# HTDerekLiu/surface_multigrid_code

Hardware: AMD Instinct MI355X
Metric: V-cycles/sec + fine-level SpMV GB/s (% HBM peak), 1M-vert mesh fp64 (higher is better)
Workload: dtype f64; 1 GPU; C3: bunny_15K_init x3 midpoint subdivision, 1011330 verts, 5 levels, M_bary+0.01(-L), fp64; n_verts=1011330, nnz=7079298, levels=5, smoother=gs, rhs_columns_per_gpu=1, parallelism=single GPU

## Files before the change

### surface_multigrid_code_amd/csrc/smg_cycle.cpp

```cpp
#include <hip/hip_runtime.h>

#include <algorithm>
#include <chrono>
#include <cmath>
#include <cstdarg>
#include <cstdio>
#include <cstdlib>
#include <cstring>
#include <functional>
#include <memory>
#include <numeric>
#include <string>
#include <thread>
#include <vector>

#include "smg_internal.hpp"

using namespace smg;


template <typename T>
static int ensure_vectors(smg_hierarchy* h, int k)
{
    constexpr bool fp64 = std::is_same<T, double>::value;
// ... 68 lines not shown
    if ((rc = prepare_sweep_plans(h, k, h->pre, h->post))) return rc;
    return ensure_spectral_bounds(h);
}

int smg::ensure_fp32(smg_hierarchy* h, int k)
{
    const int L = h->n_levels;
    if (h->union_m > 0) return fail(SMG_ERR_INVALID, "a union handle solves in fp64 (its coarse inverses are per-member blocks: no fp32 image)");
    if (h->coarse_sparse) return fail(SMG_ERR_INVALID, "the mixed-precision cycle is not available with a sparse coarse factorisation (coarsest level of %d unknowns)", h->nc);
    if (!h->f32_valid) {
        drop_graphs(h);
        for (int lv = 0; lv < L; lv++) {
            Level& Lv = h->lv[lv];
            if (lv < L - 1 && h->bs == 3) {
                HIPCHK(Lv.bA.ensure_f32(h->stream));
                if (Lv.gs_on_transpose) HIPCHK(Lv.bAT.ensure_f32(h->stream));
            } else if (lv < L - 1) {
                HIPCHK(Lv.dA.ensure_f32(h->stream));
                if (Lv.gs_on_transpose) HIPCHK(Lv.dAT.ensure_f32(h->stream));
            }
            if (lv >= 1) {
                HIPCHK(Lv.dP.ensure_f32(h->stream));
                HIPCHK(Lv.dPT.ensure_f32(h->stream));
            }
        }
        if (h->coarse_schur) {
            HIPCHK(h->sch.arena32.ensure((size_t)h->schur.off_C));
            HIPCHK(launch_cvt_f64_f32(h->sch.arena32.p, h->sch.arena.p, (size_t)h->schur.off_C, h->stream));
            h->sch.view.arena32 = h->sch.arena32.p;
        } else {
            HIPCHK(h->d_Ainv32.ensure((size_t)h->nc_pad * h->nc_pad));
            HIPCHK(launch_cvt_f64_f32(h->d_Ainv32.p, h->d_Ainv.p, (size_t)h->nc_pad * h->nc_pad, h->stream));
        }
        h->f32_valid = true;
    }
    return ensure_vectors<float>(h, k);
}

int smg::level_kind(const smg_hierarchy* h, int lv)
{
    if (lv < 0 || lv >= h->n_levels - 1) return LV_GS;
    switch (h->smoother) {
        case SMG_SMOOTH_JACOBI: return LV_JACOBI;
        case SMG_SMOOTH_HYBRID: return h->lv[lv].n <= h->jacobi_max_rows ? LV_JACOBI : LV_GS;
        case SMG_SMOOTH_CHEBYSHEV: return LV_CHEBY;
        case SMG_SMOOTH_HYBRID_CHEBYSHEV: return h->lv[lv].n <= h->jacobi_max_rows ? LV_CHEBY : LV_GS;
    }
    return LV_GS;
}

struct ChebyCoef { double c1, c2; };
static void cheby_coefs(double lam, double frac, int degree, std::vector<ChebyCoef>& out)
{
    out.resize((size_t)std::max(degree, 0));
    const double lmax = lam, lmin = lam * frac;
    const double theta = (lmax + lmin) / 2.0, delta = (lmax - lmin) / 2.0;
    const double sigma = theta / delta;
    double rho = 1.0 / sigma;
    for (int s = 0; s < degree; s++) {
        if (s == 0) { out[s].c1 = 0.0; out[s].c2 = 1.0 / theta; }
        else {
            const double rho_new = 1.0 / (2.0 * sigma - rho);
            out[s].c1 = rho_new * rho;
            out[s].c2 = 2.0 * rho_new / delta;
            rho = rho_new;
        }
    }
}

static inline int coarse_cols(const smg_hierarchy* h, int k) { return (h->coarse_cols > 0 && h->coarse_cols < k) ? h->coarse_cols : k; }


static const SellBuf& smoothed(const Level& L) { return L.gs_on_transpose ? L.dAT : L.dA; }

template <typename T>
static hipError_t coarse_solve(smg_hierarchy* h, Level& L, int k, const Ctrl* ctrl)
{
    LevelVecs<T>& V = vecs<T>(L);
    if constexpr (std::is_same<T, double>::value) {
        if (h->union_m > 0) return launch_blockdiag_gemv_add(h->un.view, h->d_Ainv.p, h->nc, V.b.p, V.u.p, k, ctrl, h->stream);
        if (h->coarse_sparse) return launch_sparse_coarse_solve(h->c_view, V.b.p, V.u.p, k, ctrl, h->stream);
    }
    if (h->coarse_schur) return launch_schur_solve(h->sch.view, V.b.p, V.u.p, k, ctrl, h->stream);
    return launch_dense_gemv_add(by_type<T>(h->d_Ainv.p, h->d_Ainv32.p), h->nc, h->nc_pad, V.b.p, V.u.p, coarse_cols(h, k), k, ctrl, h->stream, (T*)h->d_sympart.p);
}

template <typename T>
static hipError_t op_A(smg_hierarchy* h, Level& L, bool smoother_image, SellMode m, int s0, int s1, const T* x, const T* bb, T* y, int k, const Ctrl* ctrl,
                       const FirstColour* fc = nullptr, double omega = 1.0)
{
    if (h->bs == 3) {
        const Bsr3Dev& V = (smoother_image && L.gs_on_transpose) ? L.bAT.view : L.bA.view;
        return launch_bsr3(m, V, s0, s1 < 0 ? V.n_slices : s1, x, bb, y, k, ctrl, nullptr, nullptr, h->stream, omega, fc ? fc->c1 : 0.0, fc ? fc->update<T>() : nullptr);
    }
    const SellDev& V = smoother_image ? smoothed(L).view : L.dA.view;
    return launch_sell(m, V, s0, s1 < 0 ? V.n_slices : s1, x, bb, y, k, ctrl, nullptr, nullptr, h->stream, nullptr, fc, omega);
}

static const std::vector<int>& colour_slices(const smg_hierarchy* h, const Level& Lv)
{
    if (h->bs == 3) return (Lv.gs_on_transpose ? Lv.bAT : Lv.bA).color_slice_ptr;
    return (Lv.gs_on_transpose ? Lv.dAT : Lv.dA).color_slice_ptr;
}

template <typename T>
static int enqueue_gs(smg_hierarchy* h, int lv, const SweepPlan& sp, const T* b, T* u, int k, int iters, const Ctrl* ctrl, int first = FIRST_NONE, T* t = nullptr,
                      T* res = nullptr)
{
    Level& Lv = h->lv[lv];
    ProfGuard pg(h, "MG: relaxation");
    if (const WgsBuf* W = sp.wave) {
        for (int it = 0; it < iters; it++)
            for (size_t c = 0; c + 1 < W->color_ptr.size(); c++)
                HIPCHK(launch_wgs(W->view, W->color_ptr[c], W->color_ptr[c + 1], (const double*)b, (double*)u, k, ctrl, h->stream));
        return SMG_OK;
    }
    if (const BgsBuf* Q = sp.block) {
        for (int it = 0; it < iters; it++)
            for (size_t c = 0; c + 1 < Q->color_ptr.size(); c++)
                HIPCHK(launch_bgs(Q->view, Q->color_ptr[c], Q->color_ptr[c + 1], (const double*)b, (double*)u, k, ctrl, h->stream));
        return SMG_OK;
    }
    const std::vector<int>& cs = colour_slices(h, Lv);
    const SellDev& G = smoothed(Lv).view;
    FirstColour fr;
    fr.set_update(res);
    for (int it = first == FIRST_SWEEP ? 1 : 0; it < iters; it++)
        for (size_t c = (it == 0 && first == FIRST_LAUNCH) ? 1 : 0; c + 1 < cs.size(); c++) {
            const bool last = res && it == iters - 1 && c + 2 == cs.size();
            if (it == 1 && first == FIRST_SWEEP) HIPCHK(launch_sell(last ? SELL_GS_OOP_RES : SELL_GS_OOP, G, cs[c], cs[c + 1], t, b, u, k, ctrl, nullptr, nullptr, h->stream, nullptr, last ? &fr : nullptr));
            else if (last) HIPCHK(launch_sell(SELL_GS_RES, G, cs[c], cs[c + 1], u, b, u, k, ctrl, nullptr, nullptr, h->stream, nullptr, &fr));
            else HIPCHK(op_A<T>(h, Lv, true, SELL_GS, cs[c], cs[c + 1], u, b, u, k, ctrl));
        }
    return SMG_OK;
}

template <typename T>
static int enqueue_gs_tiled(smg_hierarchy* h, const TiledDev& plan, const T* b, T* const buf[2], int* cur, int k, const Ctrl* ctrl)
{
    ProfGuard pg(h, "MG: relaxation");
    HIPCHK(launch_tiled_gs(plan, (const double*)buf[*cur], (const double*)b, (double*)buf[1 - *cur], k, ctrl, h->stream));
    *cur ^= 1;
    return SMG_OK;
}

template <typename T>
static int enqueue_jacobi(smg_hierarchy* h, int lv, const T* b, T* const buf[2], int* cur, int k, int iters, const Ctrl* ctrl)
{
    Level& Lv = h->lv[lv];
    ProfGuard pg(h, "MG: relaxation");
    for (int it = 0; it < iters; it++) {
        HIPCHK(op_A<T>(h, Lv, true, SELL_JACOBI, 0, -1, buf[*cur], b, buf[1 - *cur], k, ctrl, nullptr, h->omega));
        *cur ^= 1;
    }
    return SMG_OK;
}

template <typename T>
static int enqueue_cheby(smg_hierarchy* h, int lv, const T* b, T* const buf[2], int* cur, int k, int iters, const Ctrl* ctrl, bool first_done = false)
{
    if (iters <= 0) return SMG_OK;
    Level& Lv = h->lv[lv];
    ProfGuard pg(h, "MG: relaxation");
    std::vector<ChebyCoef> cf;
    cheby_coefs(Lv.lam, h->cheby_fraction, iters + 1, cf);
    for (int s = first_done ? 1 : 0; s <= iters; s++) {
        FirstColour fc;
        fc.set_update(vecs<T>(Lv).d.p);
        fc.c1 = cf[s].c1;
        HIPCHK(op_A<T>(h, Lv, true, SELL_CHEBY, 0, -1, buf[*cur], b, buf[1 - *cur], k, ctrl, &fc, cf[s].c2));
        *cur ^= 1;
    }
    return SMG_OK;
}

static bool fuse_first_colour() { static const int on = env_int("SMG_FUSE_FIRST", 1); return on != 0; }
static bool resid_byproduct() { static const int on = env_int("SMG_RESID_BYPRODUCT", 1); return on != 0; }
static bool prolong_skip_first() { static const int on = env_int("SMG_PROLONG_SKIP_FIRST", 1); return on != 0; }

template <typename T>
static int enqueue_vcycle_t(smg_hierarchy* h, int lv, int k, int pre, int post, const Ctrl* ctrl, int first = FIRST_NONE)
{
    const bool first_done = first != FIRST_NONE;
    const int L = h->n_levels;
    Level& Lv = h->lv[lv];
    if (lv == L - 1) {
        ProfGuard pg(h, "MG: coarse solve");
        HIPCHK(coarse_solve<T>(h, Lv, k, ctrl));
        return SMG_OK;
    }
    Level& Lc = h->lv[lv + 1];
    LevelVecs<T>&V = vecs<T>(Lv), &Vc = vecs<T>(Lc);
    const int kind = level_kind(h, lv);
    const bool jac = kind != LV_GS;
    T* const buf[2] = {V.u.p, V.t.p};
    int cur = 0;
    const bool fp64 = std::is_same<T, double>::value;
    const SweepPlan sp_pre = sweep_plan(h, lv, k, pre, fp64, first), sp_post = sweep_plan(h, lv, k, post, fp64, FIRST_NONE);
    int rc;
    const bool byprod = fp64 && resid_byproduct() && h->bs == 1 && kind == LV_GS && sp_pre.colours() && pre >= 1 && k < 8 && !Lv.gs_on_transpose &&
                        Lv.dA.n_part > 0 && Lv.dA.color_slice_ptr.size() >= 3 && (first != FIRST_SWEEP || pre >= 2);
    if (kind == LV_JACOBI) {
        if (first_done) cur = 1;
        rc = enqueue_jacobi<T>(h, lv, V.b.p, buf, &cur, k, pre - (first_done ? 1 : 0), ctrl);
    } else if (kind == LV_CHEBY) {
        if (first_done) cur = 1;
        rc = enqueue_cheby<T>(h, lv, V.b.p, buf, &cur, k, pre, ctrl, first_done);
    } else if (sp_pre.tiled) rc = enqueue_gs_tiled<T>(h, *sp_pre.tiled, V.b.p, buf, &cur, k, ctrl);
    else rc = enqueue_gs<T>(h, lv, sp_pre, V.b.p, buf[0], k, pre, ctrl, first, buf[1], byprod ? V.r.p : nullptr);
    if (rc) return rc;
    {
        ProfGuard pg(h, "MG: residual");
        if (byprod) HIPCHK(launch_sell(SELL_RESID, Lv.dA.part_view(), 0, Lv.dA.n_part, buf[cur], V.b.p, V.r.p, k, ctrl, nullptr, nullptr, h->stream));
        else HIPCHK(op_A<T>(h, Lv, false, SELL_RESID, 0, -1, buf[cur], V.b.p, V.r.p, k, ctrl));
    }
    const SellBuf& Gc = smoothed(Lc);
    const int kind_c = level_kind(h, lv + 1);
    const bool jac_c = kind_c != LV_GS;
    const bool fuse = h->bs == 1 && sweep_plan(h, lv + 1, k, pre, fp64, FIRST_NONE).colours() && fuse_first_colour() && lv + 1 < L - 1 && pre > 0 && Gc.view.vals<T>() && (jac_c ? Gc.n_all > 0 : Gc.n_first > 0);
    const int kt = k * h->bs;
    {
        ProfGuard pg(h, "MG: restrict");
        FirstColour fc;
        if (fuse) {
            fc.diag_slot = Gc.diag_slot.p; fc.n_first = jac_c ? Gc.n_all : Gc.n_first;
            fc.val = Gc.view.val; fc.valf = Gc.view.valf;
            fc.jacobi = kind_c == LV_CHEBY ? 2 : (jac_c ? 1 : 0); fc.omega = h->omega;
            if (kind_c == LV_CHEBY) {
                std::vector<ChebyCoef> cf;
                cheby_coefs(Lc.lam, h->cheby_fraction, 1, cf);
                fc.omega = cf[0].c2;
                fc.set_update(Vc.d.p);
            }
        }
        T* init = (fuse && jac_c) ? Vc.t.p : Vc.u.p;
        HIPCHK(launch_sell(SELL_AX, Lc.dPT.view, 0, Lc.dPT.view.n_slices, V.r.p, nullptr, Vc.b.p, kt, ctrl, nullptr, nullptr, h->stream, init, fuse ? &fc : nullptr));
    }
    rc = enqueue_vcycle_t<T>(h, lv + 1, k, pre, post, ctrl, fuse ? FIRST_LAUNCH : FIRST_NONE);
    if (rc) return rc;
    {
        ProfGuard pg(h, "MG: prolong");
        int dst = cur;
        const int flips = sp_post.tiled ? 1 : kind == LV_CHEBY ? (post > 0 ? post + 1 : 0) : post;
        if ((jac || sp_post.tiled) && ((cur + flips) & 1)) dst = 1 - cur;
        if (!jac && !sp_post.tiled && cur == 1) dst = 0;
        const bool skip = prolong_skip_first() && h->bs == 1 && kind == LV_GS && sp_post.colours() && post >= 1 && Lc.dP.n_part > 0;
        const SellDev Pv = skip ? Lc.dP.part_view() : Lc.dP.view;
        HIPCHK(launch_sell(SELL_ADD, Pv, 0, Pv.n_slices, Vc.u.p, buf[cur], buf[dst], kt, ctrl, nullptr, nullptr, h->stream));
        cur = dst;
    }
    if (kind == LV_CHEBY) return enqueue_cheby<T>(h, lv, V.b.p, buf, &cur, k, post, ctrl);
    if (jac) return enqueue_jacobi<T>(h, lv, V.b.p, buf, &cur, k, post, ctrl);
    if (sp_post.tiled) return enqueue_gs_tiled<T>(h, *sp_post.tiled, V.b.p, buf, &cur, k, ctrl);
    return enqueue_gs<T>(h, lv, sp_post, V.b.p, buf[0], k, post, ctrl);
}

int smg::enqueue_vcycle(smg_hierarchy* h, int k, const Ctrl* ctrl, int first)
{
    if (h->precision == 1) return enqueue_vcycle_t<float>(h, 0, k, h->pre, h->post, ctrl);
    return enqueue_vcycle_t<double>(h, 0, k, h->pre, h->post, ctrl, first);
}

int smg::apply_A(smg_hierarchy* h, int lv, SellMode mode, const double* x, const double* b, double* y, int k, const Ctrl* ctrl)
{
    HIPCHK(op_A<double>(h, h->lv[lv], false, mode, 0, -1, x, b, y, k, ctrl));
    return SMG_OK;
}


template <typename T>
static int enqueue_relax(smg_hierarchy* h, int lv, const T* b, T* u, int k, int iters, const Ctrl* ctrl, T** res)
{
    const int kind = level_kind(h, lv);
    const SweepPlan sp = sweep_plan(h, lv, k, iters, std::is_same<T, double>::value, FIRST_NONE);
    T* const buf[2] = {u, vecs<T>(h->lv[lv]).t.p};
    int cur = 0, rc;
    if (kind == LV_GS && !sp.tiled) rc = enqueue_gs<T>(h, lv, sp, b, u, k, iters, ctrl);
    else if (kind == LV_GS) rc = enqueue_gs_tiled<T>(h, *sp.tiled, b, buf, &cur, k, ctrl);
    else if (kind == LV_CHEBY) rc = enqueue_cheby<T>(h, lv, b, buf, &cur, k, iters, ctrl);
    else rc = enqueue_jacobi<T>(h, lv, b, buf, &cur, k, iters, ctrl);
    *res = buf[cur];
    return rc;
}
static int enqueue_relax_into(smg_hierarchy* h, int lv, const double* b, double* u, int k, int iters, const Ctrl* ctrl)
{
    double* res = nullptr;
    int rc = enqueue_relax<double>(h, lv, b, u, k, iters, ctrl, &res);
    if (rc) return rc;
    if (res != u) HIPCHK(hipMemcpyAsync(u, res, (size_t)h->lv[lv].n * k * sizeof(double), hipMemcpyDeviceToDevice, h->stream));
    return SMG_OK;
}

bool smg::head_fusable(smg_hierarchy* h, int k)
{
    static const int on = env_int("SMG_FUSE_HEAD", 1);
    if (!on || h->precision != 0 || h->n_levels < 2 || h->prof_on || h->bs != 1 || h->union_m > 0) return false;
    Level& L0 = h->lv[0];
    if (L0.gs_on_transpose) return false;
    if (!sweep_plan(h, 0, k, h->pre, true, FIRST_NONE).colours()) return false;
    const int kind = level_kind(h, 0);
    return kind == LV_GS ? h->pre >= 2 : h->pre >= 1;
}

int smg::enqueue_residual_ss(smg_hierarchy* h, int k, bool fuse_decide, double* sumsq_out)
{
    Level& L0 = h->lv[0];
    int nb = 0;
    if (h->head_fuse) {
        ProfGuard pg(h, "MG: relaxation");
        const int kind = level_kind(h, 0);
        const SellDev& G = L0.dA.view;
        if (kind == LV_GS) {
            const std::vector<int>& cs = L0.dA.color_slice_ptr;
            for (size_t c = 0; c + 1 < cs.size(); c++) {
                int nbc = 0;
                HIPCHK(launch_sell(SELL_GS_HEAD, G, cs[c], cs[c + 1], L0.u.p, L0.b.p, L0.t.p, k, h->d_ctrl.p, h->d_partials.p + nb, &nbc, h->stream));
                nb += nbc;
            }
        } else if (kind == LV_JACOBI) {
            HIPCHK(launch_sell(SELL_JACOBI_HEAD, G, 0, G.n_slices, L0.u.p, L0.b.p, L0.t.p, k, h->d_ctrl.p, h->d_partials.p, &nb, h->stream, nullptr, nullptr, h->omega));
        } else {
            std::vector<ChebyCoef> cf;
            cheby_coefs(L0.lam, h->cheby_fraction, h->pre + 1, cf);
            FirstColour fc;
            fc.d = L0.d.p;
            fc.c1 = cf[0].c1;
            HIPCHK(launch_sell(SELL_CHEBY_HEAD, G, 0, G.n_slices, L0.u.p, L0.b.p, L0.t.p, k, h->d_ctrl.p, h->d_partials.p, &nb, h->stream, nullptr, &fc, cf[0].c2));
        }
        if (fuse_decide) HIPCHK(launch_ss_finalize_decide(h->d_partials.p, nb, h->d_ctrl.p, h->stream));
        else HIPCHK(launch_ss_finalize(h->d_partials.p, nb, h->d_ctrl.p, h->stream, sumsq_out));
        return SMG_OK;
    }
    ProfGuard pg(h, "MG: outer residual");
    if (h->union_m > 0) {
        if (!fuse_decide) return fail(SMG_ERR_INVALID, "a union handle runs through smg_solve / smg_solve_begin + smg_raw_outer_iteration (no split-phase iteration: its members stop one by one)");
        HIPCHK(launch_sell(SELL_RESID, L0.dA.view, 0, L0.dA.view.n_slices, L0.u.p, L0.b.p, L0.r.p, k, h->d_ctrl.p, nullptr, nullptr, h->stream));
        HIPCHK(launch_union_sumsq_decide(h->un.view, L0.r.p, L0.u.p, k, h->d_ctrl.p, h->stream));
        return SMG_OK;
    }
    if (h->precision == 1 && h->bs == 3)
        HIPCHK(launch_bsr3(SELL_RESID_BOTH, L0.bA.view, 0, L0.bA.view.n_slices, L0.u.p, L0.b.p, L0.r.p, k, h->d_ctrl.p, h->d_partials.p, &nb, h->stream));
    else if (h->precision == 1)
        HIPCHK(launch_sell(SELL_RESID_BOTH, L0.dA.view, 0, L0.dA.view.n_slices, L0.u.p, L0.b.p, L0.r.p, k, h->d_ctrl.p, h->d_partials.p, &nb, h->stream));
    else if (h->bs == 3)
        HIPCHK(launch_bsr3(SELL_RESID_SS, L0.bA.view, 0, L0.bA.view.n_slices, L0.u.p, L0.b.p, nullptr, k, h->d_ctrl.p, h->d_partials.p, &nb, h->stream));
    else
        HIPCHK(launch_sell(SELL_RESID_SS, L0.dA.view, 0, L0.dA.view.n_slices, L0.u.p, L0.b.p, nullptr, k, h->d_ctrl.p, h->d_partials.p, &nb, h->stream));
    if (fuse_decide) HIPCHK(launch_ss_finalize_decide(h->d_partials.p, nb, h->d_ctrl.p, h->stream));
    else HIPCHK(launch_ss_finalize(h->d_partials.p, nb, h->d_ctrl.p, h->stream, sumsq_out));
    return SMG_OK;
}

int smg::enqueue_cycle_part(smg_hierarchy* h, int k, const double* d_sumsq)
{
    if (d_sumsq) HIPCHK(launch_decide(h->d_ctrl.p, d_sumsq, h->stream));
    {
        ProfGuard pg(h, "MG: total VCycle");
        if (h->precision == 1) {
            Level& L0 = h->lv[0];
            const size_t cnt = (size_t)L0.n * k;
            HIPCHK(launch_residual_to_f32(L0.f32.b.p, L0.f32.u.p, L0.r.p, cnt, h->d_ctrl.p, h->stream));
            int rc = enqueue_vcycle(h, k, h->d_ctrl.p, FIRST_NONE);
            if (rc) return rc;
            HIPCHK(launch_add_correction(L0.u.p, L0.f32.u.p, cnt, h->d_ctrl.p, h->stream));
        } else {
            int rc = enqueue_vcycle(h, k, h->d_ctrl.p, h->head_fuse ? FIRST_SWEEP : FIRST_NONE);
            if (rc) return rc;
            if (h->union_m > 0) HIPCHK(launch_union_restore(h->un.view, h->lv[0].u.p, k, h->d_ctrl.p, h->stream));
        }
    }
    return SMG_OK;
}

int smg::coarse_stall_check(smg_hierarchy* h)
{
    if (!h->coarse_sparse || !h->c_err.p) return SMG_OK;
    int cerr = 0;
    HIPCHK(hipMemcpy(&cerr, h->c_err.p, sizeof(int), hipMemcpyDeviceToHost));
    if (!cerr) return SMG_OK;
    (void)hipMemset(h->c_err.p, 0, sizeof(int));
    return fail(SMG_ERR_HIP, "the triangular solves of the sparse coarse factorisation stalled (results are NaN)");
}

int smg::check_ready(const smg_hierarchy* h, const char* who)
{
    if (!h) return fail(SMG_ERR_INVALID, "%s: null handle", who);
    if (!h->precomputed) return fail(SMG_ERR_INVALID, "%s: call smg_precompute first", who);
    if (h->device < 0) return fail(SMG_ERR_NO_DEVICE, "%s: no HIP device", who);
    return SMG_OK;
}

int smg::internal_cols(const smg_hierarchy* h, int k)
{
    static const int on = env_int("SMG_PAD_COLS", 1);
    if (!on || k <= 4 || k > 64 || h->union_m > 0) return k;
    if (k > 32) return k > 40 ? 64 : k;
    int p = 8;
    while (p < k) p *= 2;
    return p;
}

static int piece_prolog(smg_hierarchy* h, int lv, int k, const char* who, bool need_coarser);

static int time_graph(smg_hierarchy* h, hipGraphExec_t g, int reps, double* us)
{
    hipEvent_t e0, e1;
    HIPCHK(hipEventCreate(&e0));
    HIPCHK(hipEventCreate(&e1));
    for (int i = 0; i < 3; i++) HIPCHK(hipGraphLaunch(g, h->stream));
    HIPCHK(hipEventRecord(e0, h->stream));
    for (int i = 0; i < reps; i++) HIPCHK(hipGraphLaunch(g, h->stream));
    HIPCHK(hipEventRecord(e1, h->stream));
    HIPCHK(hipStreamSynchronize(h->stream));
    float ms = 0.f;
    HIPCHK(hipEventElapsedTime(&ms, e0, e1));
    *us = 1e3 * ms / reps;
    (void)hipEventDestroy(e0); (void)hipEventDestroy(e1); (void)hipGraphExecDestroy(g);
    return SMG_OK;
}

extern "C" int smg_bench_vcycle(smg_hierarchy* h, int lv, int k, int pre, int post, int reps, double* us_per_cycle)
{
    int rc = piece_prolog(h, lv, k, "smg_bench_vcycle", false);
    if (rc) return rc;
    DeviceScope dsc(h->device);
    if (reps < 1 || !us_per_cycle) return fail(SMG_ERR_INVALID, "smg_bench_vcycle: bad arguments");
    if ((rc = prepare_sweep_plans(h, k, pre, post))) return rc;
    hipGraphExec_t g = nullptr;
    rc = capture_graph(h, &g, [&]() { return enqueue_vcycle_t<double>(h, lv, k, pre, post, nullptr); });
    if (rc) return rc;
    if ((rc = time_graph(h, g, reps, us_per_cycle))) return rc;
    return coarse_stall_check(h);
}

extern "C" int smg_bench_relax(smg_hierarchy* h, int lv, int k, int sweeps, int reps, double* us_per_call)
{
    int rc = piece_prolog(h, lv, k, "smg_bench_relax", true);
    if (rc) return rc;
    DeviceScope dsc(h->device);
    if (reps < 1 || sweeps < 1 || !us_per_call) return fail(SMG_ERR_INVALID, "smg_bench_relax: bad arguments");
    if ((rc = prepare_sweep_plans(h, k, sweeps, sweeps))) return rc;
    Level& Lv = h->lv[lv];
    hipGraphExec_t g = nullptr;
    rc = capture_graph(h, &g, [&]() { return enqueue_relax_into(h, lv, Lv.b.p, Lv.u.p, k, sweeps, nullptr); });
    if (rc) return rc;
    return time_graph(h, g, reps, us_per_call);
}

extern "C" int smg_synchronize(smg_hierarchy* h)
// ... 414 lines not shown
```

### surface_multigrid_code_amd/csrc/smg_device.hip

```cpp
#include <hip/hip_runtime.h>

#include <cstdlib>
#include <type_traits>

#include "smg_device.hpp"
#include "smg_device_inl.hpp"
#include "smg_gj_inl.hpp"

namespace smg {


__device__ int g_never_done = 0;
const int* never_done()
{
    static const int* p = nullptr;
    if (!p) { void* q = nullptr; if (hipGetSymbolAddress(&q, HIP_SYMBOL(g_never_done)) == hipSuccess) p = (const int*)q; }
    return p;
}


template <typename T> struct CoarseInit { T* u; const T* gs_val; const int* diag_slot; int n_first; int jacobi; T omega; T* d; T c1; int codes; T tab[4]; };
template <typename T> __device__ __forceinline__ T code_val(const CoarseInit<T>& z, int cw)
{
    const T lo = (cw & 1) ? z.tab[1] : z.tab[0], hi = (cw & 1) ? z.tab[3] : z.tab[2];
    return (cw & 2) ? hi : lo;
}

template <int MODE, int KB, typename T, int W0C = -1, int WPB = 4, bool CODED = false>
__global__ __launch_bounds__(64 * WPB) void k_sell(const int* a_col, const T* a_val, const int* a_order, const int* a_slice_off, int a_stride,
                                              int a_w_lo, int s_begin, int s_end, int n_blocks, int use_order, const T* x,
                                              const int* a_slice_row, const int* a_slice_w, const T* b, T* y, int ld, const int* done,
                                              double* partials, CoarseInit<T> z)
{
    struct { const int *slice_row, *slice_off, *slice_w, *order, *col; int stride, w_lo; } A = {a_slice_row, a_slice_off, a_slice_w, a_order,
                                                                                               a_col, a_stride, a_w_lo};
    constexpr int C = 64;
    const int lane = threadIdx.x & 63;
    const int wave = threadIdx.x >> 6;
    constexpr int wpb = WPB;
    constexpr bool GS = sell_is_gs(MODE), OOP = sell_is_oop(MODE), JAC = sell_is_jacobi(MODE), CHEB = sell_is_cheby(MODE), HEAD = sell_is_head(MODE);
    constexpr bool RES = sell_has_res(MODE);
    int bid;
    if (GS && n_blocks < 0) { if (blockIdx.x & 7) return; bid = blockIdx.x >> 3; }
    else bid = xcd_remap(blockIdx.x, n_blocks);
    const int ls = __builtin_amdgcn_readfirstlane(s_begin + bid * wpb + wave);
    double ss = 0.0;
    int stop = 0;
    if (ls < s_end) {
        const int s = (!GS && use_order) ? A.order[ls] : ls;
        const int W0 = W0C >= 0 ? W0C : (A.w_lo < 8 ? A.w_lo : 8);
        const int off0 = (W0C >= 0 || A.stride) ? s * A.stride : A.slice_off[s];
        const int* cp = A.col + (size_t)off0 * C + lane;
        const T* vp = CODED ? nullptr : a_val + (size_t)off0 * C + lane;
        constexpr int U = W0C > 8 ? W0C : 8;
        int c0[U];
        T v0[U];
#pragma unroll
        for (int t = 0; t < U; t++) {
            if (t < W0) { c0[t] = cp[(size_t)t * C]; v0[t] = CODED ? (T)0 : vp[(size_t)t * C]; }
            else { c0[t] = -1; v0[t] = (T)0; }
        }
        {
            size_t keep = (size_t)x ^ (size_t)A.slice_row ^ (size_t)A.slice_w ^ (size_t)b ^ (size_t)y ^ (size_t)done ^ (size_t)ld;
            if (MODE == SELL_AX) keep ^= (size_t)z.u ^ (size_t)z.gs_val ^ (size_t)z.diag_slot ^ (size_t)z.n_first ^ (size_t)z.jacobi ^ (size_t)z.d;
            if (CHEB || RES) keep ^= (size_t)z.d;
            asm("" : "+s"(keep));
            if (keep == 0x5a5a5a5a5a5a5a5bull) return;
        }
        stop = load_flag(done);
        const int row0 = A.slice_row[s];
        const int nrow = A.slice_row[s + 1] - row0;
        const int w = A.slice_w[s];
        const int rowb = row0 + lane;
        const int split = OOP ? A.slice_row[s_begin] : 0;
        T acc[KB];
        T accr[KB];
        T diag = (T)1;
        T xi[KB];
        T dold[KB];
        T bv[KB];
        const bool live = lane < nrow;
        T zd = (T)1;
        if (MODE == SELL_AX && live && rowb < z.n_first) zd = z.gs_val[z.diag_slot[rowb]];
#pragma unroll
        for (int q = 0; q < KB; q++) {
            acc[q] = (T)0; accr[q] = (T)0; xi[q] = (T)0; dold[q] = (T)0;
            if (MODE == SELL_AX) bv[q] = (T)0;
            else bv[q] = live ? b[(size_t)rowb * ld + q] : (T)0;
            if (CHEB && live && z.c1 != (T)0) dold[q] = z.d[(size_t)rowb * ld + q];
        }
        bool has_diag = false;
        auto consume = [&](const int (&cw)[U], const T (&vw)[U]) {
            int c[U];
            T v[U];
#pragma unroll
            for (int t = 0; t < U; t++) {
                if constexpr (CODED) { c[t] = cw[t] >> 2; v[t] = code_val<T>(z, cw[t]); }
                else { c[t] = cw[t]; v[t] = vw[t]; }
            }
            T xv[U][KB];
            T xo[MODE == SELL_GS_HEAD ? U : 1][KB];
#pragma unroll
            for (int t = 0; t < U; t++) {
                const bool use = (c[t] >= 0) && !(GS && c[t] == rowb);
                if constexpr (MODE == SELL_GS_HEAD) {
                    gather_kb<KB, T>(x + (size_t)c[t] * ld, c[t] >= 0, xo[t]);
                    gather_kb<KB, T>((const T*)y + (size_t)c[t] * ld, use && c[t] < split, xv[t]);
                } else if constexpr (MODE == SELL_GS_OOP || MODE == SELL_GS_OOP_RES) {
                    gather_kb<KB, T>((c[t] < split ? (const T*)y : x) + (size_t)c[t] * ld, use, xv[t]);
                } else {
                    gather_kb<KB, T>(x + (size_t)c[t] * ld, use, xv[t]);
                }
            }
#pragma unroll
            for (int t = 0; t < U; t++) {
                if (c[t] >= 0) {
                    if (HEAD) {
#pragma unroll
                        for (int q = 0; q < KB; q++) accr[q] += v[t] * (MODE == SELL_GS_HEAD ? xo[t][q] : xv[t][q]);
                    }
                    if (GS && c[t] == rowb) {
                        diag = v[t];
                        if (RES) has_diag = true;
                    } else if ((JAC || CHEB) && c[t] == rowb) {
// ... 413 lines not shown
        else if (A.w_max <= 16) SMG_WIDE_LAT(16);
        else SMG_WIDE_LAT(32);
#undef SMG_WIDE_LAT
        *nb_out = nb;
        return;
    }
    const int waves = ns * (KW / 2);
    const int nb = (waves + 3) / 4;
    hipLaunchKernelGGL((k_sell_wide<MODE, KW, T>), dim3(nb), dim3(256), 0, st, A.col, A.vals<T>(), A.order, A.slice_off, A.stride, s_begin, s_end, nb, use_order, x,
                       A.slice_row, A.slice_w, b, y, k, done, partials, zero_rows);
    *nb_out = nb;
}

int sell_wide_blocks(int n_slices, int k)
{
    int tot = 0, c0 = 0;
    while (k - c0 >= 8) { int kw = 64; while (kw > k - c0) kw >>= 1; tot += (n_slices * kw + 3) / 4; c0 += kw; }
    return tot;
}

static constexpr int sell_wpb() { return 4; }
static int gs_wpb() { static const int v = getenv("SMG_GS_WPB") ? atoi(getenv("SMG_GS_WPB")) : 4; return v; }
int sell_blocks(int n_slices) { return (n_slices + sell_wpb() - 1) / sell_wpb(); }

template <typename T>
struct NarrowRun {
    int s_begin, s_end, use_order;
    const T *xx, *bb;
    T* yy;
    int k;
    const int* done;
    double* pp;
    const CoarseInit<T>& zz;
    hipStream_t st;
};
template <int MODE, int KB, typename T, int W0C, int WPB, bool CODED>
static void narrow_one(const SellDev& A, int grid, int nbarg, const NarrowRun<T>& R)
{
    hipLaunchKernelGGL((k_sell<MODE, KB, T, W0C, WPB, CODED>), dim3(grid), dim3(64 * WPB), 0, R.st, A.col, CODED ? nullptr : A.vals<T>(), A.order, A.slice_off, A.stride, A.w_lo,
                       R.s_begin, R.s_end, nbarg, R.use_order, R.xx, A.slice_row, A.slice_w, R.bb, R.yy, R.k, R.done, R.pp, R.zz);
}
template <int MODE, typename T, bool CODED>
static void launch_narrow(const SellDev& A, int kb, int nb, int ns, int grid, int nbarg, bool one_xcd, const NarrowRun<T>& R)
{
    static_assert(sell_wpb() == 4, "the narrow kernels below are instantiated for 4 waves per workgroup");
    const bool w7 = A.stride > 0 && A.w_lo == 7;
    switch (kb) {
        case 1: {
            const int w0 = A.stride > 0 ? (A.w_lo < 8 ? A.w_lo : 8) : -1;
            static const int pitch_env = getenv("SMG_PITCH_SPEC_MAX") ? atoi(getenv("SMG_PITCH_SPEC_MAX")) : -1;
            const int pitch_max = pitch_env >= 0 ? pitch_env : (sell_is_gs(MODE) ? 32 : 64);
            if (nb <= pitch_max && A.stride == 12 && w0 >= 7) narrow_one<MODE, 1, T, 12, 4, CODED>(A, grid, nbarg, R);
            else if (!CODED && w0 == 7 && MODE == SELL_GS && !one_xcd && gs_wpb() == 8) narrow_one<SELL_GS, 1, T, 7, 8, false>(A, (ns + 7) / 8, (ns + 7) / 8, R);
            else if (!CODED && w0 == 7 && MODE == SELL_GS && !one_xcd && gs_wpb() == 2) narrow_one<SELL_GS, 1, T, 7, 2, false>(A, (ns + 1) / 2, (ns + 1) / 2, R);
            else if (w0 == 7) narrow_one<MODE, 1, T, 7, 4, CODED>(A, grid, nbarg, R);
            else if (w0 == 8) narrow_one<MODE, 1, T, 8, 4, CODED>(A, grid, nbarg, R);
            else if (w0 == 2) narrow_one<MODE, 1, T, 2, 4, CODED>(A, grid, nbarg, R);
            else narrow_one<MODE, 1, T, -1, 4, CODED>(A, grid, nbarg, R);
            break;
        }
        case 2:
            if (w7) narrow_one<MODE, 2, T, 7, 4, CODED>(A, grid, nbarg, R);
            else narrow_one<MODE, 2, T, -1, 4, CODED>(A, grid, nbarg, R);
            break;
        case 3:
            if (w7) narrow_one<MODE, 3, T, 7, 4, CODED>(A, grid, nbarg, R);
            else narrow_one<MODE, 3, T, -1, 4, CODED>(A, grid, nbarg, R);
            break;
        default:
            if (w7) narrow_one<MODE, 4, T, 7, 4, CODED>(A, grid, nbarg, R);
            else narrow_one<MODE, 4, T, -1, 4, CODED>(A, grid, nbarg, R);
            break;
    }
}

template <int MODE, typename T>
static hipError_t launch_sell_mode(const SellDev& A, int s_begin, int s_end_in, const T* x, const T* b, T* y,
                                   int k, const Ctrl* ctrl, double* partials, int* n_blocks, hipStream_t st, T* zero_rows, const FirstColour* first,
                                   double omega)
{
    int s_end = s_end_in;
    if (MODE == SELL_ADD && !b) b = y;
    if constexpr (sell_has_res(MODE)) { if (k >= 8 || !first || !first->d || zero_rows || s_end_in != A.n_slices) return hipErrorInvalidValue; }
    const int ns = s_end - s_begin;
    const int nb = sell_blocks(ns);
    const int* done = ctrl ? &ctrl->done : never_done();
    static const int dbg_empty = getenv("SMG_DEBUG_EMPTY") ? atoi(getenv("SMG_DEBUG_EMPTY")) : 0;
    if (dbg_empty == 1) s_end = s_begin;
    const int use_order = (A.order && s_begin == 0 && s_end == A.n_slices) ? 1 : 0;
    if (n_blocks) *n_blocks = 0;
    if (ns <= 0) return hipSuccess;
    int c0 = 0;
    size_t poff = 0;
    if constexpr (!sell_has_res(MODE)) {
        while (k - c0 >= 8) {
            int kw = 64;
            while (kw > k - c0) kw >>= 1;
            const T* xx = x ? x + c0 : nullptr;
            const T* bb = b ? b + c0 : nullptr;
            T* yy = y ? y + c0 : nullptr;
            double* pp = partials ? partials + poff : nullptr;
            const CoarseInit<T> zz = coarse_codes<T>(A, zero_rows, c0, first, omega);
            int wnb = 0;
            switch (kw) {
                case 64: launch_wide_one<MODE, 64, T>(A, s_begin, s_end, use_order, xx, bb, yy, k, done, pp, zz, st, &wnb); break;
                case 32: launch_wide_one<MODE, 32, T>(A, s_begin, s_end, use_order, xx, bb, yy, k, done, pp, zz, st, &wnb); break;
                case 16: launch_wide_one<MODE, 16, T>(A, s_begin, s_end, use_order, xx, bb, yy, k, done, pp, zz, st, &wnb); break;
                default: launch_wide_one<MODE, 8, T>(A, s_begin, s_end, use_order, xx, bb, yy, k, done, pp, zz, st, &wnb); break;
            }
            poff += (size_t)wnb;
            c0 += kw;
        }
    }
    static const int one_xcd_max = getenv("SMG_ONE_XCD_MAX") ? atoi(getenv("SMG_ONE_XCD_MAX")) : 32;
    const bool one_xcd = sell_is_gs(MODE) && nb <= one_xcd_max;
    const int grid = one_xcd ? nb * 8 : nb, nbarg = one_xcd ? -nb : nb;
    for (; c0 < k; c0 += 4) {
        const int kb = (k - c0) < 4 ? (k - c0) : 4;
        const T* xx = x ? x + c0 : nullptr;
        const T* bb = b ? b + c0 : nullptr;
        T* yy = y ? y + c0 : nullptr;
        double* pp = partials ? partials + poff : nullptr;
        const CoarseInit<T> zz = coarse_codes<T>(A, zero_rows, c0, first, omega);
        poff += (size_t)nb;
        if constexpr (std::is_same<T, double>::value && (MODE == SELL_AX || MODE == SELL_RESID)) {
            int kd = kb;
            if (kd == 4 && !deep_wanted(MODE, A.w_max, 4) && deep_wanted(MODE, A.w_max, 2)) kd = 2;
            if (deep_wanted(MODE, A.w_max, kd) || (kd > 1 && deep_wanted(MODE, A.w_max, 1))) {
                for (int cc = 0; cc < kb;) {
                    int kk = kb - cc;
                    while (kk > 1 && !deep_wanted(MODE, A.w_max, kk)) kk--;
                    const int nbm = A.w_max <= 24 ? 3 : A.w_max <= 40 ? 5 : 8;
                    const CoarseInit<T> zc = coarse_codes<T>(A, zero_rows, c0 + cc, first, omega);
#define SMG_DEEP_LAUNCH(KB, NB) hipLaunchKernelGGL((k_sell_deep<MODE, KB, NB>), dim3(nb), dim3(256), 0, st, A.col, A.val, A.order, A.slice_off, A.stride, s_begin, s_end, nb, use_order, \
                                                   xx ? xx + cc : nullptr, A.slice_row, A.slice_w, bb ? bb + cc : nullptr, yy + cc, k, done, zc)
                    if (nbm == 3) { if (kk == 1) SMG_DEEP_LAUNCH(1, 3); else if (kk == 2) SMG_DEEP_LAUNCH(2, 3); else SMG_DEEP_LAUNCH(3, 3); }
                    else if (nbm == 5) { if (kk == 1) SMG_DEEP_LAUNCH(1, 5); else SMG_DEEP_LAUNCH(2, 5); }
                    else SMG_DEEP_LAUNCH(1, 8);
#undef SMG_DEEP_LAUNCH
                    cc += kk;
                }
                continue;
            }
        }
        const NarrowRun<T> run{s_begin, s_end, use_order, xx, bb, yy, k, done, pp, zz, st};
        if constexpr (MODE == SELL_AX || MODE == SELL_ADD) {
            if (A.codes) { launch_narrow<MODE, T, true>(A, kb, nb, ns, grid, nbarg, one_xcd, run); continue; }
        }
        launch_narrow<MODE, T, false>(A, kb, nb, ns, grid, nbarg, one_xcd, run);
    }
    if (MODE == SELL_AX && A.long_n > 0 && s_begin == 0 && s_end_in == A.n_slices && A.long_vals<T>()) {
        const CoarseInit<T> zz = coarse_codes<T>(A, zero_rows, 0, first, omega);
        if (k >= 8) {
            const long waves = (long)A.long_n * ((k + 63) / 64);
            hipLaunchKernelGGL((k_long_ax_cols<T>), dim3((unsigned)((waves + 3) / 4)), dim3(256), 0, st, A.long_row, A.long_ptr, A.long_col, A.long_vals<T>(), A.long_n, x, y,
                               k, k, done, zz);
        } else {
            const long waves = (long)A.long_n * k;
            hipLaunchKernelGGL((k_long_ax<T>), dim3((unsigned)((waves + 3) / 4)), dim3(256), 0, st, A.long_row, A.long_ptr, A.long_col, A.long_vals<T>(), A.long_n, x, y, k, k,
                               done, zz);
        }
    }
    if (n_blocks) *n_blocks = (int)poff;
    return hipGetLastError();
}

template <typename T>
static hipError_t launch_sell_any(SellMode mode, const SellDev& A, int s_begin, int s_end, const T* x, const T* b,
                                  T* y, int k, const Ctrl* ctrl, double* partials, int* n_blocks, hipStream_t st,
                                  T* zero_rows, const FirstColour* first, double omega)
{
    constexpr bool fp64 = std::is_same<T, double>::value;
    if (!fp64 && ((!A.valf && !A.codes) || partials)) return hipErrorInvalidValue;
    switch (mode) {
#define SMG_SELL_CASE(M) \
        case M: \
            if constexpr (fp64 || !sell_fp64_only(M)) return launch_sell_mode<M, T>(A, s_begin, s_end, x, b, y, k, ctrl, partials, n_blocks, st, zero_rows, first, omega); \
            else return hipErrorInvalidValue;
        SMG_SELL_CASE(SELL_JACOBI) SMG_SELL_CASE(SELL_CHEBY) SMG_SELL_CASE(SELL_AX) SMG_SELL_CASE(SELL_RESID) SMG_SELL_CASE(SELL_RESID_SS)
        SMG_SELL_CASE(SELL_ADD) SMG_SELL_CASE(SELL_GS) SMG_SELL_CASE(SELL_RESID_BOTH) SMG_SELL_CASE(SELL_GS_OOP) SMG_SELL_CASE(SELL_GS_HEAD)
        SMG_SELL_CASE(SELL_JACOBI_HEAD) SMG_SELL_CASE(SELL_CHEBY_HEAD) SMG_SELL_CASE(SELL_GS_RES) SMG_SELL_CASE(SELL_GS_OOP_RES)
#undef SMG_SELL_CASE
    }
    return hipErrorInvalidValue;
}

hipError_t launch_sell(SellMode mode, const SellDev& A, int s_begin, int s_end, const double* x, const double* b,
                       double* y, int k, const Ctrl* ctrl, double* partials, int* n_blocks, hipStream_t st,
                       double* zero_rows, const FirstColour* first, double omega)
{
    return launch_sell_any<double>(mode, A, s_begin, s_end, x, b, y, k, ctrl, partials, n_blocks, st, zero_rows, first, omega);
}
hipError_t launch_sell(SellMode mode, const SellDev& A, int s_begin, int s_end, const float* x, const float* b,
                       float* y, int k, const Ctrl* ctrl, double* partials, int* n_blocks, hipStream_t st,
                       float* zero_rows, const FirstColour* first, double omega)
{
    return launch_sell_any<float>(mode, A, s_begin, s_end, x, b, y, k, ctrl, partials, n_blocks, st, zero_rows, first, omega);
}

__global__ __launch_bounds__(256) void k_gershgorin(const int* a_col, const double* a_val, const int* a_slice_row, const int* a_slice_off, const int* a_slice_w,
                                                    int stride, int n_slices, unsigned long long* out)
{
    const int lane = threadIdx.x & 63, s = blockIdx.x * 4 + (threadIdx.x >> 6);
    double ratio = 0.0;
    if (s < n_slices) {
        const int row0 = a_slice_row[s], nrow = a_slice_row[s + 1] - row0, w = a_slice_w[s];
        const size_t off = (size_t)(stride ? s * stride : a_slice_off[s]) * 64 + lane;
        double sum = 0.0, diag = 0.0;
        for (int j = 0; j < w; j++) {
            const int c = a_col[off + (size_t)j * 64];
            const double v = a_val[off + (size_t)j * 64];
            if (c >= 0) { sum += fabs(v); if (c == row0 + lane) diag = v; }
        }
        if (lane < nrow && diag > 0.0) ratio = sum / diag;
    }
#pragma unroll
    for (int o = 32; o > 0; o >>= 1) ratio = fmax(ratio, __shfl_down(ratio, o, 64));
    if (lane == 0 && ratio > 0.0) atomicMax(out, (unsigned long long)__double_as_longlong(ratio));
}
hipError_t launch_gershgorin(const SellDev& A, double* out, hipStream_t st)
{
    hipError_t e = hipMemsetAsync(out, 0, sizeof(double), st);
    if (e != hipSuccess || A.n_slices <= 0) return e;
    hipLaunchKernelGGL(k_gershgorin, dim3((A.n_slices + 3) / 4), dim3(256), 0, st, A.col, A.val, A.slice_row, A.slice_off, A.slice_w, A.stride, A.n_slices,
                       (unsigned long long*)out);
    return hipGetLastError();
}


__global__ __launch_bounds__(256) void k_ss_finalize(const double* partials, int n, Ctrl* ctrl, double* out)
{
    if (ctrl->done) return;
    __shared__ double red[256];
    double s = 0.0;
    for (int i = threadIdx.x; i < n; i += 256) s += partials[i];
    red[threadIdx.x] = s;
    __syncthreads();
    for (int o = 128; o > 0; o >>= 1) {
        if ((int)threadIdx.x < o) red[threadIdx.x] += red[threadIdx.x + o];
        __syncthreads();
    }
    if (threadIdx.x == 0) *out = red[0];
}

__global__ __launch_bounds__(256) void k_ss_finalize_decide(const double* partials, int n, Ctrl* ctrl)
{
    __shared__ double red[256];
    const int done = ctrl->done, n_his = ctrl->n_his, his_cap = ctrl->his_cap;
    const double tol = ctrl->tol;
    double* const r_his = ctrl->r_his;
    double s = 0.0;
#pragma unroll 8
    for (int i = threadIdx.x; i < n; i += 256) s += partials[i];
    if (done) return;
    red[threadIdx.x] = s;
    __syncthreads();
    for (int o = 128; o > 0; o >>= 1) {
        if ((int)threadIdx.x < o) red[threadIdx.x] += red[threadIdx.x + o];
        __syncthreads();
    }
    if (threadIdx.x == 0) {
        const double sumsq = red[0], r = sqrt(sumsq);
        ctrl->sumsq = sumsq;
        if (n_his < his_cap) r_his[n_his] = r;
        ctrl->n_his = n_his + 1;
        ctrl->r_prev = ctrl->r_last; ctrl->r_last = r;
        if (!(r == r) || r > 1.7e308) { ctrl->status = -1; ctrl->done = 1; }
        else if (r < tol) ctrl->done = 1;
    }
}

__global__ void k_decide(Ctrl* ctrl, const double* sumsq)
{
    if (ctrl->done) return;
    decide_body(ctrl, *sumsq);
}

constexpr int SS_STAGE_MIN = 16384, SS_STAGE_WGS = 128;
__global__ __launch_bounds__(256) void k_ss_stage(const double* __restrict__ partials, int n, double* __restrict__ out, const int* done)
{
    if (load_flag(done)) return;
    __shared__ double red[256];
    const int per = (n + SS_STAGE_WGS - 1) / SS_STAGE_WGS;
    const int i0 = blockIdx.x * per, i1 = min(n, i0 + per);
    double s = 0.0;
#pragma unroll 8
    for (int i = i0 + (int)threadIdx.x; i < i1; i += 256) s += partials[i];
    red[threadIdx.x] = s;
    __syncthreads();
    for (int o = 128; o > 0; o >>= 1) {
        if ((int)threadIdx.x < o) red[threadIdx.x] += red[threadIdx.x + o];
        __syncthreads();
    }
    if (threadIdx.x == 0) out[blockIdx.x] = red[0];
}
static const double* ss_stage(const double* partials, int& n, const Ctrl* ctrl, hipStream_t st)
{
    if (n < SS_STAGE_MIN) return partials;
    double* out = const_cast<double*>(partials) + n;
    hipLaunchKernelGGL(k_ss_stage, dim3(SS_STAGE_WGS), dim3(256), 0, st, partials, n, out, &ctrl->done);
    n = SS_STAGE_WGS;
    return out;
}
int ss_partials_room() { return SS_STAGE_WGS; }

hipError_t launch_ss_finalize(const double* partials, int n, Ctrl* ctrl, hipStream_t st, double* out)
{
    partials = ss_stage(partials, n, ctrl, st);
    hipLaunchKernelGGL(k_ss_finalize, dim3(1), dim3(256), 0, st, partials, n, ctrl, out ? out : &ctrl->sumsq);
    return hipGetLastError();
}
__global__ void k_decide_spec(Ctrl* ctrl, const double* sumsq)
{
    ctrl->just_done = 0;
    if (ctrl->done) return;
    decide_body(ctrl, *sumsq);
    if (ctrl->done) ctrl->just_done = 1;
}
__global__ void k_copy_unless_done(double* dst, const double* src, size_t n, const int* done)
{
    if (*done) return;
    const size_t i = (size_t)blockIdx.x * blockDim.x + threadIdx.x;
    if (i < n) dst[i] = src[i];
}
__global__ void k_restore_if_just_done(double* dst, const double* src, size_t n, const Ctrl* ctrl)
{
    if (!ctrl->just_done) return;
    const size_t i = (size_t)blockIdx.x * blockDim.x + threadIdx.x;
    if (i < n) dst[i] = src[i];
}
hipError_t launch_decide_spec(Ctrl* ctrl, const double* sumsq, hipStream_t st)
{
    hipLaunchKernelGGL(k_decide_spec, dim3(1), dim3(1), 0, st, ctrl, sumsq);
    return hipGetLastError();
}
hipError_t launch_copy_unless_done(double* dst, const double* src, size_t n, const Ctrl* ctrl, hipStream_t st)
{
    if (n == 0) return hipSuccess;
    hipLaunchKernelGGL(k_copy_unless_done, dim3((unsigned)((n + 255) / 256)), dim3(256), 0, st, dst, src, n, &ctrl->done);
    return hipGetLastError();
}
hipError_t launch_restore_if_just_done(double* dst, const double* src, size_t n, const Ctrl* ctrl, hipStream_t st)
{
    if (n == 0) return hipSuccess;
    hipLaunchKernelGGL(k_restore_if_just_done, dim3((unsigned)((n + 255) / 256)), dim3(256), 0, st, dst, src, n, ctrl);
    return hipGetLastError();
}
hipError_t launch_ss_finalize_decide(const double* partials, int n, Ctrl* ctrl, hipStream_t st)
{
    partials = ss_stage(partials, n, ctrl, st);
    hipLaunchKernelGGL(k_ss_finalize_decide, dim3(1), dim3(256), 0, st, partials, n, ctrl);
    return hipGetLastError();
}
hipError_t launch_decide(Ctrl* ctrl, const double* sumsq, hipStream_t st)
{
    hipLaunchKernelGGL(k_decide, dim3(1), dim3(1), 0, st, ctrl, sumsq);
    return hipGetLastError();
}

template <typename T> struct Vec2;
template <> struct Vec2<double> { typedef double type __attribute__((ext_vector_type(2))); };
template <> struct Vec2<float> { typedef float type __attribute__((ext_vector_type(2))); };

template <int KB, typename T>
__global__ __launch_bounds__(256) void k_dense_gemv_add(const T* __restrict__ Ainv, int n, int lda,
                                                        const T* __restrict__ b, T* u, int ld, const int* done)
{
    const int stop = load_flag(done);
    const int lane = threadIdx.x & 63;
    const int row = blockIdx.x * 4 + (threadIdx.x >> 6);
    if (row >= n) return;
    using T2 = typename Vec2<T>::type;
    const T2* a2 = reinterpret_cast<const T2*>(Ainv + (size_t)row * lda);
    T acc[KB];
#pragma unroll
    for (int q = 0; q < KB; q++) acc[q] = (T)0;
    const int n2 = lda >> 1;
#pragma unroll 4
    for (int jj = lane; jj < n2; jj += 64) {
        const T2 a = a2[jj];
#pragma unroll
        for (int q = 0; q < KB; q++) {
            acc[q] += a.x * b[(size_t)(2 * jj) * ld + q];
            acc[q] += a.y * b[(size_t)(2 * jj + 1) * ld + q];
        }
    }
#pragma unroll
// ... 142 lines not shown
            for (int c = 0; c < CPW; c++) bn[c][t] = (q < per && col0 + 16 * c + lc < kvalid) ? pb[q * sb + 16 * c] : 0.0;
        }
#pragma unroll
        for (int t = 0; t < DEPTH; t++)
#pragma unroll
            for (int c = 0; c < CPW; c++) acc[c] = __builtin_amdgcn_mfma_f64_16x16x4f64(av[t], bv[c][t], acc[c], 0, 0, 0);
#pragma unroll
        for (int t = 0; t < DEPTH; t++) {
            av[t] = an[t];
#pragma unroll
            for (int c = 0; c < CPW; c++) bv[c][t] = bn[c][t];
        }
    }
    __shared__ double red[CPW][4][4][64];
#pragma unroll
    for (int c = 0; c < CPW; c++)
#pragma unroll
        for (int r = 0; r < 4; r++) red[c][w][r][lane] = acc[c][r];
    __syncthreads();
    if (!stop) {
        for (int c = w; c < CPW; c += 4) {
#pragma unroll
            for (int r = 0; r < 4; r++) {
                const int row = row0 + lr + 4 * r;
                if (row < n && col0 + 16 * c + lc < kvalid) {
                    const size_t o = (size_t)row * ld + col0 + 16 * c + lc;
                    u[o] = u[o] + ((red[c][0][r][lane] + red[c][1][r][lane]) + (red[c][2][r][lane] + red[c][3][r][lane]));
                }
            }
        }
    }
}

template <typename T>
__global__ __launch_bounds__(256) void k_sym_gemv_tiles(const T* __restrict__ Ainv, int lda, const T* __restrict__ b, T* __restrict__ part, int nb)
{
    const int idx = blockIdx.x;
    int I = (int)((sqrtf(8.0f * (float)idx + 1.0f) - 1.0f) * 0.5f);
    I -= (I * (I + 1) / 2 > idx);
    I += ((I + 1) * (I + 2) / 2 <= idx);
    const int J = idx - I * (I + 1) / 2;
    __shared__ T tile[64][65];
    __shared__ T bI[64], bJ[64];
    const int t = threadIdx.x;
#pragma unroll
    for (int e = 0; e < 16; e++) {
        const int idx = e * 256 + t, r = idx >> 6, c = idx & 63;
        tile[r][c] = Ainv[(size_t)(I * 64 + r) * lda + J * 64 + c];
    }
    if (t < 64) bJ[t] = b[J * 64 + t];
    else if (t < 128) bI[t - 64] = b[I * 64 + t - 64];
    __syncthreads();
    __shared__ T red[4][64];
    const int g = t >> 6, l = t & 63, h0 = (g & 1) * 32;
    T s = (T)0;
    if (g < 2) {
#pragma unroll 8
        for (int c = h0; c < h0 + 32; c++) s += tile[l][c] * bJ[c];
    } else {
#pragma unroll 8
        for (int r = h0; r < h0 + 32; r++) s += tile[r][l] * bI[r];
    }
    red[g][l] = s;
    __syncthreads();
    if (t < 64) part[((size_t)I * nb + J) * 64 + t] = red[0][t] + red[1][t];
    else if (t < 128 && I != J) part[((size_t)J * nb + I) * 64 + (t - 64)] = red[2][t - 64] + red[3][t - 64];
}
template <typename T>
__global__ __launch_bounds__(256) void k_sym_gemv_sum(const T* __restrict__ part, int nb, int n, T* u, const int* done)
{
    const int stop = load_flag(done);
    __shared__ T red[4][64];
    const int a = blockIdx.x, g = threadIdx.x >> 6, l = threadIdx.x & 63;
    const int q = (nb + 3) / 4, b0 = g * q, b1 = min(nb, b0 + q);
    T s = (T)0;
#pragma unroll 8
    for (int bidx = b0; bidx < b1; bidx++) s += part[((size_t)a * nb + bidx) * 64 + l];
    red[g][l] = s;
    __syncthreads();
    const int i = a * 64 + l;
    if (g == 0 && i < n && !stop) u[i] = u[i] + ((red[0][l] + red[1][l]) + (red[2][l] + red[3][l]));
}

template <typename T>
static hipError_t launch_dense_T(const T* Ainv, int n, int lda, const T* b, T* u, int k, int ld, const Ctrl* ctrl, hipStream_t st, void* sym_work)
{
    const int* done = ctrl ? &ctrl->done : never_done();
    const int nb = (n + 3) / 4;
    if (n <= 0) return hipSuccess;
    if (k == 1 && ld == 1 && sym_work && lda % 64 == 0 && lda >= 512) {
        const int nt = lda / 64;
        hipLaunchKernelGGL((k_sym_gemv_tiles<T>), dim3(nt * (nt + 1) / 2), dim3(256), 0, st, Ainv, lda, b, (T*)sym_work, nt);
        hipLaunchKernelGGL((k_sym_gemv_sum<T>), dim3(nt), dim3(256), 0, st, (const T*)sym_work, nt, n, u, done);
        return hipGetLastError();
    }
    int c0 = 0;
    static const int use_mfma8 = getenv("SMG_COARSE_MFMA") ? atoi(getenv("SMG_COARSE_MFMA")) : 1;
    const int mfma_min = (std::is_same<T, double>::value && use_mfma8 && lda % 64 == 0) ? 8 : 16;
    while (k - c0 >= mfma_min) {
        int kc = 64;
        while (kc > k - c0 && kc > 16) kc >>= 1;
        const int kv = kc < k - c0 ? kc : k - c0;
        const int tb = (n + 15) / 16;
        static const int use_mfma = getenv("SMG_COARSE_MFMA") ? atoi(getenv("SMG_COARSE_MFMA")) : 1;
        if constexpr (std::is_same<T, double>::value) {
            if (use_mfma && lda % 64 == 0) {
                static const int cpw = getenv("SMG_COARSE_CPW") ? atoi(getenv("SMG_COARSE_CPW")) : 2;
                if (kc == 64 && cpw == 2) { hipLaunchKernelGGL((k_dense_gemm_mfma_multi<64, 2>), dim3(tb * 2), dim3(256), 0, st, Ainv, n, lda, b + c0, u + c0, ld, done, kv); c0 += kv; continue; }
                switch (kc) {
                    case 64: hipLaunchKernelGGL((k_dense_gemm_mfma<64>), dim3(tb * 4), dim3(256), 0, st, Ainv, n, lda, b + c0, u + c0, ld, done, kv); break;
                    case 32: hipLaunchKernelGGL((k_dense_gemm_mfma<32>), dim3(tb * 2), dim3(256), 0, st, Ainv, n, lda, b + c0, u + c0, ld, done, kv); break;
                    default: hipLaunchKernelGGL((k_dense_gemm_mfma<16>), dim3(tb), dim3(256), 0, st, Ainv, n, lda, b + c0, u + c0, ld, done, kv); break;
                }
                c0 += kv;
                continue;
            }
        }
        switch (kc) {
            case 64: hipLaunchKernelGGL((k_dense_gemm_tile<64, T>), dim3(tb), dim3(256), 0, st, Ainv, n, lda, b + c0, u + c0, ld, done); break;
            case 32: hipLaunchKernelGGL((k_dense_gemm_tile<32, T>), dim3(tb), dim3(256), 0, st, Ainv, n, lda, b + c0, u + c0, ld, done); break;
            default: hipLaunchKernelGGL((k_dense_gemm_tile<16, T>), dim3(tb), dim3(256), 0, st, Ainv, n, lda, b + c0, u + c0, ld, done); break;
        }
        c0 += kc;
    }
    for (; c0 < k; c0 += 4) {
        const int kb = (k - c0) < 4 ? (k - c0) : 4;
        switch (kb) {
            case 1: hipLaunchKernelGGL((k_dense_gemv_add<1, T>), dim3(nb), dim3(256), 0, st, Ainv, n, lda, b + c0, u + c0, ld, done); break;
            case 2: hipLaunchKernelGGL((k_dense_gemv_add<2, T>), dim3(nb), dim3(256), 0, st, Ainv, n, lda, b + c0, u + c0, ld, done); break;
            case 3: hipLaunchKernelGGL((k_dense_gemv_add<3, T>), dim3(nb), dim3(256), 0, st, Ainv, n, lda, b + c0, u + c0, ld, done); break;
            default: hipLaunchKernelGGL((k_dense_gemv_add<4, T>), dim3(nb), dim3(256), 0, st, Ainv, n, lda, b + c0, u + c0, ld, done); break;
        }
    }
    return hipGetLastError();
}
template <typename T>
static hipError_t launch_sym_tiles_T(const T* Ainv, int lda, const T* b, T* part, hipStream_t st)
{
    if (lda <= 0 || lda % 64) return hipErrorInvalidValue;
    const int nt = lda / 64;
    hipLaunchKernelGGL((k_sym_gemv_tiles<T>), dim3(nt * (nt + 1) / 2), dim3(256), 0, st, Ainv, lda, b, part, nt);
    return hipGetLastError();
}
hipError_t launch_sym_gemv_tiles(const double* Ainv, int lda, const double* b, double* part, hipStream_t st) { return launch_sym_tiles_T<double>(Ainv, lda, b, part, st); }
hipError_t launch_sym_gemv_tiles(const float* Ainv, int lda, const float* b, float* part, hipStream_t st) { return launch_sym_tiles_T<float>(Ainv, lda, b, part, st); }
hipError_t launch_dense_gemv_add(const double* Ainv, int n, int lda, const double* b, double* u, int k, int ld,
                                 const Ctrl* ctrl, hipStream_t st, double* sym_work)
{
    return launch_dense_T<double>(Ainv, n, lda, b, u, k, ld, ctrl, st, sym_work);
}
hipError_t launch_dense_gemv_add(const float* Ainv, int n, int lda, const float* b, float* u, int k, int ld,
                                 const Ctrl* ctrl, hipStream_t st, float* sym_work)
{
    return launch_dense_T<float>(Ainv, n, lda, b, u, k, ld, ctrl, st, sym_work);
}

__global__ void k_cvt_f64_f32(float* dst, const double* src, size_t n)
{
    const size_t i = (size_t)blockIdx.x * blockDim.x + threadIdx.x;
    if (i < n) dst[i] = (float)src[i];
}
__global__ void k_residual_to_f32(float* b32, float* u32, const double* r64, size_t n, const int* done)
{
    if (done && *done) return;
    const size_t i = (size_t)blockIdx.x * blockDim.x + threadIdx.x;
    if (i < n) { b32[i] = (float)r64[i]; u32[i] = 0.0f; }
}
__global__ void k_add_correction(double* z, const float* e, size_t n, const int* done)
{
    if (done && *done) return;
    const size_t i = (size_t)blockIdx.x * blockDim.x + threadIdx.x;
    if (i < n) z[i] = z[i] + (double)e[i];
}
hipError_t launch_cvt_f64_f32(float* dst, const double* src, size_t n, hipStream_t st)
{
    if (n == 0) return hipSuccess;
    hipLaunchKernelGGL(k_cvt_f64_f32, dim3((unsigned)((n + 255) / 256)), dim3(256), 0, st, dst, src, n);
    return hipGetLastError();
}
hipError_t launch_residual_to_f32(float* b32, float* u32, const double* r64, size_t n, const Ctrl* ctrl, hipStream_t st)
{
    if (n == 0) return hipSuccess;
    hipLaunchKernelGGL(k_residual_to_f32, dim3((unsigned)((n + 255) / 256)), dim3(256), 0, st, b32, u32, r64, n, ctrl ? &ctrl->done : nullptr);
    return hipGetLastError();
}
hipError_t launch_add_correction(double* z, const float* e, size_t n, const Ctrl* ctrl, hipStream_t st)
{
    if (n == 0) return hipSuccess;
    hipLaunchKernelGGL(k_add_correction, dim3((unsigned)((n + 255) / 256)), dim3(256), 0, st, z, e, n, ctrl ? &ctrl->done : nullptr);
    return hipGetLastError();
}

constexpr int GJ_H = 32;

__global__ __launch_bounds__(256) void k_gj_diag(const double* M, int n, int kb, double* dinv)
{
    __shared__ double a[GJ_NB][GJ_NB + 1];
    __shared__ double Rb[16][GJ_NB + 1];
    __shared__ double Cb[GJ_NB][17];
    const int K = kb * GJ_NB;
    for (int e = threadIdx.x; e < GJ_NB * GJ_NB; e += 256) a[e / GJ_NB][e % GJ_NB] = M[(size_t)(K + e / GJ_NB) * n + K + e % GJ_NB];
    __syncthreads();
    gj_invert64(a, Rb, Cb);
    for (int e = threadIdx.x; e < GJ_NB * GJ_NB; e += 256) dinv[e] = a[e / GJ_NB][e % GJ_NB];
}

__global__ __launch_bounds__(256) void k_gj_panels(const double* M, int n, int kb, const double* dinv, double* rowp,
                                                   double* colp)
{
    __shared__ double m_s[GJ_NB][GJ_H + 1];
    const int K = kb * GJ_NB;
    const int j0 = blockIdx.x * GJ_H;
    const int J = j0 / GJ_NB;
    const int t = threadIdx.x;
    if (J == kb) {
        for (int e = t; e < GJ_NB * GJ_H; e += 256) {
            const int r = e / GJ_H, c = e % GJ_H;
            rowp[(size_t)r * n + j0 + c] = dinv[r * GJ_NB + j0 + c - K];
        }
        return;
    }
    const int lane = t & 63, w = t >> 6, lr = lane >> 4, lc = lane & 15;
    double av[GJ_NB / 4], mr[8];
#pragma unroll
    for (int q = 0; q < GJ_NB / 4; q++) av[q] = dinv[(16 * w + lc) * GJ_NB + 4 * q + lr];
    if (J < kb) {
#pragma unroll
        for (int e = 0; e < 8; e++) { const int x = t + 256 * e; mr[e] = M[(size_t)(K + x / GJ_H) * n + j0 + x % GJ_H]; }
#pragma unroll
        for (int e = 0; e < 8; e++) { const int x = t + 256 * e; m_s[x / GJ_H][x % GJ_H] = mr[e]; }
    } else {
#pragma unroll
        for (int e = 0; e < 8; e++) { const int x = t + 256 * e; mr[e] = M[(size_t)(j0 + x / GJ_NB) * n + K + x % GJ_NB]; }
#pragma unroll
        for (int e = 0; e < 8; e++) { const int x = t + 256 * e; m_s[x % GJ_NB][x / GJ_NB] = mr[e]; }
    }
    __syncthreads();
// ... 607 lines not shown
```

### surface_multigrid_code_amd/csrc/smg_device.hpp

```cpp
#pragma once
#include <hip/hip_runtime_api.h>

#include <cstdint>
#include <type_traits>

namespace smg {

template <typename T, typename D, typename F>
constexpr auto by_type(D d, F f) { if constexpr (std::is_same<T, double>::value) return d; else return f; }

struct Ctrl {
    int done;
    int n_his;
    int status;
    int just_done;
    double sumsq;
    double tol;
    double* r_his;
    int his_cap;
    int pad_;
    double r_last, r_prev;
};

struct SellDev {
    int n_rows = 0, n_cols = 0, n_slices = 0;
    int C = 64;
    const int* slice_row = nullptr;
    const int* slice_off = nullptr;
    const int* slice_w = nullptr;
    int stride = 0;
    int w_lo = 0;
    int w_max = 0;
    const int* order = nullptr;
    const int* col = nullptr;
    const double* val = nullptr;
    const float* valf = nullptr;
    int codes = 0;
    double tab[4] = {0.0, 0.0, 0.0, 0.0};
    float tabf[4] = {0.0f, 0.0f, 0.0f, 0.0f};
    int long_n = 0;
    const int* long_row = nullptr;
    const int* long_ptr = nullptr;
    const int* long_col = nullptr;
    const double* long_val = nullptr;
    const float* long_valf = nullptr;
    template <typename T> const T* vals() const { return by_type<T>(val, valf); }
    template <typename T> const T* long_vals() const { return by_type<T>(long_val, long_valf); }
    template <typename T> const T* table() const { return by_type<T>(tab, tabf); }
};

enum SellMode {
    SELL_AX = 0,
    SELL_RESID = 1,
    SELL_RESID_SS = 2,
    SELL_ADD = 3,
    SELL_GS = 4,
    SELL_RESID_BOTH = 5,
    SELL_JACOBI = 6,
    SELL_CHEBY = 7,
    SELL_GS_OOP = 8,
    SELL_GS_HEAD = 9,
    SELL_JACOBI_HEAD = 10,
    SELL_CHEBY_HEAD = 11,
    SELL_GS_RES = 12,
    SELL_GS_OOP_RES = 13,
};
constexpr bool sell_has_res(int m) { return m == SELL_GS_RES || m == SELL_GS_OOP_RES; }
constexpr bool sell_is_gs(int m) { return m == SELL_GS || m == SELL_GS_OOP || m == SELL_GS_HEAD || sell_has_res(m); }
constexpr bool sell_is_oop(int m) { return m == SELL_GS_OOP || m == SELL_GS_HEAD || m == SELL_GS_OOP_RES; }
constexpr bool sell_is_jacobi(int m) { return m == SELL_JACOBI || m == SELL_JACOBI_HEAD; }
constexpr bool sell_is_cheby(int m) { return m == SELL_CHEBY || m == SELL_CHEBY_HEAD; }
constexpr bool sell_is_head(int m) { return m == SELL_GS_HEAD || m == SELL_JACOBI_HEAD || m == SELL_CHEBY_HEAD; }
constexpr bool sell_has_ss(int m) { return sell_is_head(m) || m == SELL_RESID_SS || m == SELL_RESID_BOTH; }
constexpr bool sell_fp64_only(int m) { return sell_has_ss(m) || sell_is_oop(m) || sell_has_res(m); }

struct FirstColour {
    const int* diag_slot = nullptr;
    int n_first = 0;
    const double* val = nullptr;
    const float* valf = nullptr;
    int jacobi = 0;
    double omega = 1.0;
    double* d = nullptr;
    float* df = nullptr;
    double c1 = 0.0;
    template <typename T> const T* vals() const { return by_type<T>(val, valf); }
    template <typename T> T* update() const { return by_type<T>(d, df); }
    template <typename T> void set_update(T* p) { if constexpr (std::is_same<T, double>::value) d = p; else df = p; }
};
hipError_t launch_sell(SellMode mode, const SellDev& A, int s_begin, int s_end, const double* x, const double* b,
                       double* y, int k, const Ctrl* ctrl, double* partials, int* n_blocks, hipStream_t st,
                       double* zero_rows = nullptr, const FirstColour* first = nullptr, double omega = 1.0);
hipError_t launch_sell(SellMode mode, const SellDev& A, int s_begin, int s_end, const float* x, const float* b,
                       float* y, int k, const Ctrl* ctrl, double* partials, int* n_blocks, hipStream_t st,
                       float* zero_rows = nullptr, const FirstColour* first = nullptr, double omega = 1.0);
hipError_t launch_gershgorin(const SellDev& A, double* out, hipStream_t st);
struct Bsr3Dev {
    int n_vert = 0, n_slices = 0, w_max = 0;
    const int* slice_row = nullptr;
    const int* slice_off = nullptr;
    const int* slice_w = nullptr;
    const int* order = nullptr;
    const int* col = nullptr;
    const double* val = nullptr;
    const float* valf = nullptr;
    template <typename T> const T* vals() const { return by_type<T>(val, valf); }
};
hipError_t launch_bsr3(SellMode mode, const Bsr3Dev& A, int s_begin, int s_end, const double* x, const double* b, double* y, int k, const Ctrl* ctrl,
                       double* partials, int* n_blocks, hipStream_t st, double omega = 1.0, double c1 = 0.0, double* dvec = nullptr);
hipError_t launch_bsr3(SellMode mode, const Bsr3Dev& A, int s_begin, int s_end, const float* x, const float* b, float* y, int k, const Ctrl* ctrl,
                       double* partials, int* n_blocks, hipStream_t st, double omega = 1.0, double c1 = 0.0, float* dvec = nullptr);
hipError_t launch_bsr3_gershgorin(const Bsr3Dev& A, double* out, hipStream_t st);
int bsr3_blocks(int n_slices);
hipError_t launch_bsr3_fill(const int* ptr, const int* col, const double* val, const int* gptr, const int* gcol, const int* perm, const int* iperm, const Bsr3Dev& B,
                            size_t panel_cols, bool transposed, hipStream_t st);

struct BgsDev {
    int n_blocks = 0, n_colors = 0, xrows = 0;
    const int* hdr = nullptr;
    const int* xrow = nullptr;
    const int* ugrow = nullptr;
    const int* ulrow = nullptr;
    const double* udiag = nullptr;
    const int* eidx = nullptr;
    const double* eval = nullptr;
};
hipError_t launch_bgs(const BgsDev& P, int b_begin, int b_end, const double* b, double* u, int k, const Ctrl* ctrl, hipStream_t st);

struct WgsDev {
    int n_pieces = 0, n_colors = 0, rim_pitch = 0, nb_max = 0;
    const int* hdr = nullptr;
    const int* grow = nullptr;
    const int* meta = nullptr;
    const double* diag = nullptr;
    const int* rim = nullptr;
    const unsigned* eoff = nullptr;
    const double* eval = nullptr;
};
hipError_t launch_wgs(const WgsDev& P, int q_begin, int q_end, const double* b, double* u, int k, const Ctrl* ctrl, hipStream_t st);

struct UnionDev {
    int m = 0, his_cap = 0, max_rows = 0;
    const int* rows = nullptr;
    const int* rptr = nullptr;
    const int* crow_member = nullptr;
    const long long* moff = nullptr;
    const int* mlda = nullptr;
    const int* mrow0 = nullptr;
    double* ss = nullptr;
    double* his = nullptr;
    int* nhis = nullptr;
    int* done = nullptr;
    double* zsave = nullptr;
};
hipError_t launch_blockdiag_gemv_add(const UnionDev& U, const double* Ainv, int n, const double* b, double* u, int k, const Ctrl* ctrl, hipStream_t st);
hipError_t launch_union_sumsq_decide(const UnionDev& U, const double* r, const double* u, int k, Ctrl* ctrl, hipStream_t st);
hipError_t launch_union_restore(const UnionDev& U, double* u, int k, const Ctrl* ctrl, hipStream_t st);
hipError_t launch_scatter_dense(double* dense, const double* src, const long long* pos, int nnz, hipStream_t st);
hipError_t launch_dense_identity(double* dense, int np, int n, hipStream_t st);

struct TiledDev {
    int n_tiles = 0, nc = 0, P = 0, sweeps = 0, max_ext = 0, w_max = 0, threads = 512;
    const int* hdr = nullptr;
    const int* ext_rows = nullptr;
    const int* pcol = nullptr;
    const double* pval = nullptr;
    const int* prow = nullptr;
    const double* pdiag = nullptr;
};
hipError_t launch_tiled_gs(const TiledDev& T, const double* x, const double* b, double* y, int k, const Ctrl* ctrl, hipStream_t st);
hipError_t tiled_gs_prepare(int max_ext);

struct SparseCholDev {
    int n = 0;
    const int* perm = nullptr;
    const int *rptr = nullptr, *rcol = nullptr;
    const int *cptr = nullptr, *crow = nullptr;
    const double *rval = nullptr, *cval = nullptr, *diag = nullptr;
    double* work = nullptr;
    int* err = nullptr;
};
hipError_t launch_sparse_coarse_solve(const SparseCholDev& F, const double* b, double* u, int k, const Ctrl* ctrl, hipStream_t st);
int sparse_coarse_work_cols(int k);

constexpr int SCHUR_M_MAX_DEV = 128;
struct SchurDev {
    int n = 0, nb = 0, ns = 0, ns_pad = 0;
    const int *irow = nullptr, *bsize = nullptr, *srow = nullptr, *sptr = nullptr, *sidx = nullptr, *aptr = nullptr, *ablk = nullptr, *apan = nullptr;
    double* arena = nullptr;
    float* arena32 = nullptr;
    long long off_D = 0, off_P = 0, off_W = 0, off_S = 0, off_C = 0;
    const long long *coff = nullptr, *pos = nullptr, *pos2 = nullptr, *ones = nullptr, *rdst = nullptr, *rdst2 = nullptr, *rsrc = nullptr;
    const int* rptr = nullptr;
    int nnz = 0, n_ones = 0, n_red = 0;
    double *g = nullptr, *xs = nullptr;
    float *g32 = nullptr, *xs32 = nullptr;
    double* sym_work = nullptr;
    double* gj_work = nullptr;
    template <typename T> const T* factors() const { return by_type<T>(arena, arena32); }
    template <typename T> T* rhs() const { return by_type<T>(g, g32); }
    template <typename T> T* sol() const { return by_type<T>(xs, xs32); }
};
hipError_t launch_schur_factor(const SchurDev& F, const double* vals, hipStream_t st);
hipError_t launch_schur_check(const SchurDev& F, int* d_flag, hipStream_t st);
hipError_t launch_schur_solve(const SchurDev& F, const double* b, double* u, int k, const Ctrl* ctrl, hipStream_t st);
hipError_t launch_schur_solve(const SchurDev& F, const float* b, float* u, int k, const Ctrl* ctrl, hipStream_t st);

int sell_blocks(int n_slices);
int sell_wide_blocks(int n_slices, int k);

int ss_partials_room();
hipError_t launch_ss_finalize(const double* partials, int n, Ctrl* ctrl, hipStream_t st, double* out = nullptr);
hipError_t launch_decide(Ctrl* ctrl, const double* sumsq, hipStream_t st);
hipError_t launch_decide_spec(Ctrl* ctrl, const double* sumsq, hipStream_t st);
hipError_t launch_copy_unless_done(double* dst, const double* src, size_t n, const Ctrl* ctrl, hipStream_t st);
hipError_t launch_restore_if_just_done(double* dst, const double* src, size_t n, const Ctrl* ctrl, hipStream_t st);
hipError_t launch_ss_finalize_decide(const double* partials, int n, Ctrl* ctrl, hipStream_t st);

enum { KS_RZ = 0, KS_RZ_PREV = 1, KS_ALPHA = 2, KS_BETA = 3, KS_SLOTS = 4 };
constexpr int KRY_MAX_GROUPS = 512;
struct KryDev {
    int n = 0, k = 0;
    int groups = 0;
    double* part = nullptr;
    double* s = nullptr;
    int* restart = nullptr;
};
int kry_groups(int n, int k);
hipError_t launch_kry_dots_zr_zq(const KryDev& K, const double* z, const double* r, const double* q, const Ctrl* ctrl, hipStream_t st);
hipError_t launch_kry_direction(const KryDev& K, const double* z, double* p, const Ctrl* ctrl, hipStream_t st);
hipError_t launch_kry_dots_pq(const KryDev& K, const double* p, const double* q, const Ctrl* ctrl, hipStream_t st);
hipError_t launch_kry_step_decide(const KryDev& K, double* x, double* r, const double* p, const double* q, Ctrl* ctrl, hipStream_t st);
hipError_t launch_kry_precond_in(const double* r, double* b0, double* u0, size_t cnt, const Ctrl* ctrl, hipStream_t st);
hipError_t launch_kry_widen(const float* e, double* z, size_t cnt, const Ctrl* ctrl, hipStream_t st);
hipError_t launch_kry_arm(const KryDev& K, Ctrl* ctrl, bool reopen, hipStream_t st);

struct EigBlocks {
    const double* p[3] = {nullptr, nullptr, nullptr};
    int nb = 0;
};
constexpr int EIG_TILE = 64;
constexpr int EIG_MAX_GROUPS = 256;
int eig_groups(int n);
size_t eig_gram_part_size(int a, int b, int groups);
hipError_t launch_eig_gram(const EigBlocks& Sa, const EigBlocks& Sb, int n, int m, const double* w, bool sym, double* part, int groups,
                           double* G, const Ctrl* ctrl, hipStream_t st);
hipError_t launch_eig_combine(const EigBlocks& S, const EigBlocks& AS, int n, int m, const double* C, double* X, double* AX, double* P,
                              double* AP, const Ctrl* ctrl, hipStream_t st);
hipError_t launch_eig_residual(const double* X, const double* AX, const double* mass, const double* lam, int n, int m, double* b0, double* u0,
                               float* b32, float* u32, double* part, int groups, double* res, const Ctrl* ctrl, hipStream_t st);

hipError_t launch_dense_gemv_add(const double* Ainv, int n, int lda, const double* b, double* u, int k, int ld,
                                 const Ctrl* ctrl, hipStream_t st, double* sym_work = nullptr);
hipError_t launch_dense_gemv_add(const float* Ainv, int n, int lda, const float* b, float* u, int k, int ld,
                                 const Ctrl* ctrl, hipStream_t st, float* sym_work = nullptr);
hipError_t launch_sym_gemv_tiles(const double* Ainv, int lda, const double* b, double* part, hipStream_t st);
hipError_t launch_sym_gemv_tiles(const float* Ainv, int lda, const float* b, float* part, hipStream_t st);
hipError_t launch_cvt_f64_f32(float* dst, const double* src, size_t n, hipStream_t st);
hipError_t launch_residual_to_f32(float* b32, float* u32, const double* r64, size_t n, const Ctrl* ctrl, hipStream_t st);
hipError_t launch_add_correction(double* z, const float* e, size_t n, const Ctrl* ctrl, hipStream_t st);
hipError_t launch_spd_inverse(double* M, int n, double* work, hipStream_t st);

hipError_t launch_recipe(int n_out, const int* ptr, const int* idx, const double* coef, const double* src, double* out, hipStream_t st);
hipError_t launch_sell_fill(const int* ptr, const int* col, const double* val, const int* perm, const int* iperm, const SellDev& S, size_t padded, hipStream_t st,
                            bool transposed = false);
hipError_t launch_sell_encode(const SellDev& S, size_t padded, const double* tab, int n_tab, int* out_col, int* bad, hipStream_t st);
hipError_t launch_sell_diag_slots(const SellDev& S, int* slot, int* first_missing, hipStream_t st);
hipError_t warm_device_code(hipStream_t st);
hipError_t launch_sell_fill_map(const int* ptr, const int* col, const int* perm, const int* iperm, const SellDev& S, size_t padded, bool transposed, int* map, hipStream_t st);
hipError_t launch_bit_symmetric(int n, const int* ptr, const int* col, const double* val, int* differs, hipStream_t st);
hipError_t launch_gather_vals(double* dst, const double* src, const int* map, size_t n, hipStream_t st);
hipError_t launch_dense_from_csr(double* dense, int np, int n, const double* src, const long long* pos, int nnz, hipStream_t st);
hipError_t launch_add_at(double* v, const int* where, int n, double c, hipStream_t st);

hipError_t launch_assemble(int nV, int nF, int nnz, const double* V, const int* F, int voronoi, const int* l_ptr, const int* l_idx,
                           const signed char* l_sgn, const int* m_ptr, const int* m_idx, const int* diag_of, double* Qc, double* Qm,
                           double* Md, double mass_coef, double lap_coef, double* val, double* Lval, hipStream_t st);

hipError_t launch_gather_in(double* dst, const double* src, const int* map, int n, int k, int kin, int ld_src,
                            hipStream_t st);
hipError_t launch_scatter_out(double* dst, const double* src, const int* map, int n, int k, int kin, int ld_dst,
                              hipStream_t st);
hipError_t launch_scatter_cm(double* dst, const double* src, const int* idx, int n, int k, int ld_src, int ld_dst,
                             hipStream_t st);
hipError_t launch_gather_cm(double* dst, const double* src, const int* idx, int n, int k, int ld_src, int ld_dst,
                            hipStream_t st);
hipError_t launch_csr_sub(int n_rows, const int* ptr, const int* col, const double* val, const double* x, int ldx,
                          double* y, int ld, int k, hipStream_t st);

hipError_t launch_geo_basis(const double* V, const int* F, int nF, double* W, double* Af, hipStream_t st);
hipError_t launch_geo_scatter(int n, int k, const int* src_ptr, const int* src, double* B, int ldb, hipStream_t st);
hipError_t launch_geo_divergence(int n, int k, const int* F, const double* W, const double* Af, const int* m_ptr, const int* m_idx,
                                 const double* U, int ldu, double* out, int ldo, hipStream_t st);
hipError_t launch_geo_shift(int n, int k, const int* src_ptr, const int* src, const double* phi, int ldp, double* mean, double* D, int ldd,
                            hipStream_t st);

hipError_t launch_arap_covariance(int n, const int* rowptr, const int* col, const double* w, const double* P0, const double* P, double* S, hipStream_t st);
hipError_t launch_arap_rotations(int n, const int* rowptr, const int* col, const double* w, const double* P0, const double* P, double* R, double* eterm,
                                 hipStream_t st);
hipError_t launch_arap_vertex_energy(int n, const int* rowptr, const int* col, const double* w, const double* P0, const double* P, const double* R,
                                     double* eterm, hipStream_t st);
hipError_t launch_arap_rhs(int n, const int* rowptr, const int* col, const double* w, const double* P0, const double* R, double* B, int ldb, hipStream_t st);
hipError_t launch_arap_rows(int n, const double* U, int ldu, double* P, hipStream_t st);
hipError_t launch_arap_columns(int n, const double* P, double* U, int ldu, hipStream_t st);
hipError_t launch_arap_set_handles(int nh, const int* handles, const double* hp, int ldh, double* U, int ldu, hipStream_t st);

int fixed_sum_groups(int n);
hipError_t launch_fixed_sum(const double* term, int n, double* part, double* sum, hipStream_t st);

hipError_t launch_membrane_rest(int nF, const int* F, const double* V0, double thickness, double* rest, hipStream_t st);
hipError_t launch_membrane_faces(int mode, int nF, const int* F, const double* P, const double* rest, double alpha, double beta, double floor,
                                 double value, double* W, double* G, double* H, hipStream_t st);
hipError_t launch_membrane_matrix(int nB, const int* brow, const int* bcol, const int* bptr, const int* c_ptr, const int* c_src, const double* H,
                                  int nF, double dt2, const double* mass0, double mass_scale, double* val, hipStream_t st);
hipError_t launch_membrane_pressure(int nV, int nF, const int* F, const double* P, const int* m_ptr, const int* m_idx, double pressure, double* Qn,
                                    double* mass, double* fext, hipStream_t st);
hipError_t launch_membrane_gradient(int nV, const int* m_ptr, const int* m_idx, const double* G, int nF, const double* mass0, double mass_scale,
                                    double dt, const double* qdot, const double* qdot0, const double* fext, double* g, double* b, hipStream_t st);
hipError_t launch_membrane_trial(int nV, const double* qdot, const double* dx, double step, const double* qdot0, const double* pos0,
                                 const double* fext, const double* mass0, double mass_scale, double dt, double* t_out, double* p_out, double* term,
                                 hipStream_t st);
hipError_t launch_membrane_dot3(int nV, const double* a, const double* b, double* term, hipStream_t st);

}
```

### surface_multigrid_code_amd/csrc/smg_hier.hpp

```cpp
#pragma once
#include <memory>
#include <hip/hip_runtime_api.h>

#include <atomic>
#include <cstdint>
#include <string>
#include <vector>

#include "smg_bsr3.hpp"
#include "smg_coarse.hpp"
#include "smg_device.hpp"
#include "smg_mesh.hpp"
#include "smg_order.hpp"
#include "smg_sparse.hpp"
#include "smg_tiled.hpp"
#include "smg_bgs.hpp"
#include "smg_wgs.hpp"
#include "smg_schur.hpp"

namespace smg {

inline std::atomic<long long>& devbuf_live_bytes() { static std::atomic<long long> v{0}; return v; }

template <typename T>
// ... 163 lines not shown
    BgsBuf bgs;
    std::vector<int> A_int_src;
    DevBuf<double> d_Aval;
    DevBuf<double> d_Tval;
    DevBuf<int> mapA, mapAT;
    DevBuf<int> r1_ptr, r1_idx, r2_ptr, r2_idx;
    DevBuf<double> r1_coef, r2_coef;
    int nnzT = 0;
    LevelVecs<float> f32;
    double lam = 0.0;
    int n = 0;
};

struct GraphKey {
    int k = 0, k_user = 0, pre = 0, post = 0, precision = 0, smoother = 0, jacobi_max_rows = 0;
    double omega = 0.0, cheby_fraction = 0.0;
    bool head_fuse = false;
    bool operator==(const GraphKey& o) const
    {
        return k == o.k && k_user == o.k_user && pre == o.pre && post == o.post && precision == o.precision && smoother == o.smoother &&
               jacobi_max_rows == o.jacobi_max_rows && omega == o.omega && cheby_fraction == o.cheby_fraction && head_fuse == o.head_fuse;
    }
    bool operator!=(const GraphKey& o) const { return !(*this == o); }
};

enum Step { STEP_ITER,
            STEP_ITER_N,
            STEP_HEAD,
            STEP_TAIL,
            STEP_SPLIT_RESID,
            STEP_SPLIT_CYCLE,
            STEP_SPEC,
            STEP_PCG,
            STEP_PCG_N,
            STEP_COUNT };

struct GraphCache {
    hipGraphExec_t exec[STEP_COUNT] = {};
    GraphKey mg_key, pcg_key;
    double* sumsq = nullptr;
    void drop(int s0 = 0, int s1 = STEP_COUNT)
    {
        for (int s = s0; s < s1; s++) if (exec[s]) { (void)hipGraphExecDestroy(exec[s]); exec[s] = nullptr; }
        if (s0 <= STEP_ITER && s1 > STEP_ITER) mg_key = GraphKey();
        if (s0 <= STEP_PCG && s1 > STEP_PCG) pcg_key = GraphKey();
    }
};

template <typename T> inline LevelVecs<T>& vecs(Level& L) { if constexpr (std::is_same<T, double>::value) return L; else return L.f32; }
template <typename T> inline const LevelVecs<T>& vecs(const Level& L) { if constexpr (std::is_same<T, double>::value) return L; else return L.f32; }

struct ProfScope { std::string name; long count = 0; double ms = 0.0; };
struct ProfRec { int scope; hipEvent_t e0, e1; };

}

struct smg_hierarchy {
    int n_levels = 0;
    std::vector<smg::Level> lv;
    int n_full = 0;
    bool has_known = false, precomputed = false;
    std::vector<int> known, unknown;
    smg::Csr LHS_unused;
    smg::Csr Auk;
    smg::DevBuf<int> d_map0;
    smg::DevBuf<int> d_perm0;
    smg::DevBuf<int> d_unknown, d_known;
    smg::DevBuf<int> d_auk_ptr, d_auk_col;
    smg::DevBuf<double> d_auk_val;
    uint64_t pre_key = 0;
    int p_version = 0;
    bool input_canonical = false;
    bool recipes_built = false, host_stale = false;
    int nnz_input = 0;
    std::vector<int> lhs_src, auk_src;
    smg::DevBuf<int> d_lhs_src, d_auk_src, d_diag_idx;
    smg::DevBuf<long long> d_dense_pos;
    smg::DevBuf<double> d_Afull;
    struct EarlyUpload { smg::DevBuf<int> ptr, col; smg::DevBuf<double> val; bool valid = false; } early0;
    int nc = 0, nc_pad = 0;
    smg::DevBuf<double> d_Ainv;
    smg::DevBuf<float> d_Ainv32;
    smg::DevBuf<double> d_sympart;
    bool coarse_sparse = false;
    int coarse_dense_max = 16384;
    bool coarse_dense_max_user = false;
    bool mem_lean = false;
    int wgs_mode = -1;
    int bgs_min_rows = -1;
    smg::SparseChol chol;
    smg::DevBuf<int> c_perm, c_rptr, c_rcol, c_cptr, c_crow, c_err;
    smg::DevBuf<double> c_rval, c_cval, c_diag, c_work;
    smg::SparseCholDev c_view;
    bool coarse_schur = false;
    int coarse_schur_when = 2;
    int coarse_schur_min = 2048;
    int coarse_schur_big = 6144;
    int coarse_schur_max = 65536;
    bool schur_declined = false;
    smg::SchurPlan schur;
    struct SchurBuf {
        smg::DevBuf<int> irow, bsize, srow, sptr, sidx, aptr, ablk, acol, rptr;
        smg::DevBuf<long long> coff, pos, pos2, ones, rdst, rdst2, rsrc;
        smg::DevBuf<double> arena, g, xs, sym, gj;
        smg::DevBuf<float> arena32, g32, xs32;
        smg::SchurDev view;
        void release() { *this = SchurBuf(); }
        template <typename T> smg::DevBuf<T>& rhs() { if constexpr (std::is_same<T, double>::value) return g; else return g32; }
        template <typename T> smg::DevBuf<T>& sol() { if constexpr (std::is_same<T, double>::value) return xs; else return xs32; }
    } sch;
    bool f32_valid = false;
    int kcap32 = 0;
    int block_mode = -1;
    int bs = 1;
    int union_m = 0;
    std::vector<int> union_off0;
    std::vector<int> union_offc;
    std::vector<long long> union_moff;
    std::vector<int> union_mlda;
    struct UnionBuf {
        smg::DevBuf<int> rows, rptr, crow_member, mlda, mrow0, nhis, done;
        smg::DevBuf<long long> moff;
        smg::DevBuf<double> ss, his, zsave;
        smg::UnionDev view;
    } un;
    int device = -1;
    hipStream_t stream = nullptr;
    bool own_stream = false, user_stream = false;
    hipStream_t aux[3] = {nullptr, nullptr, nullptr};
    smg::DevBuf<smg::Ctrl> d_ctrl;
    smg::Ctrl host_ctrl;
    smg::DevBuf<double> d_rhis;
    smg::PinBuf<smg::Ctrl> pin_ctrl;
    smg::PinBuf<double> pin_his;
    smg::PinBuf<double> pin_vec;
    smg::DevBuf<double> d_partials;
    int kcap = 0;
    bool in_solve = false;
    int k = 0;
    int k_user = 0;
    int coarse_cols = 0;
    double tol = 1e-3;
    int max_iter = 20, pre = 2, post = 2, verbosity = 0, check_every = 1, use_graph = 1, precision = 0;
    int smoother = 0;
    double omega = 0.8;
    int jacobi_max_rows = 100000;
    double cheby_fraction = 0.1;
    smg::DevBuf<double> d_lam;
    bool lam_valid = false;
    int iters_enqueued = 0;
    smg::DevBuf<double> d_stage_rhs, d_stage_z, d_stage_kv, d_tmp_cm;
    smg::DevBuf<double> d_zsave;
    const double* cur_kv = nullptr;
    int cur_ld_kv = 0;
    smg::GraphCache graphs;
    bool head_fuse = false;
    smg::DevBuf<double> kry_x, kry_r, kry_p, kry_q, kry_b;
    smg::DevBuf<double> kry_part, kry_s;
    smg::DevBuf<int> kry_restart;
    smg::KryDev kry;
    smg::DevBuf<double> eig_x[2], eig_ax[2], eig_p[2], eig_ap[2];
    smg::DevBuf<double> eig_w, eig_aw;
    smg::DevBuf<double> eig_mass;
    smg::DevBuf<double> eig_part, eig_small;
    smg::DevBuf<double> eig_stage;
    smg::PinBuf<double> eig_pin;
// ... 6 lines not shown
```

### surface_multigrid_code_amd/csrc/smg_internal.hpp

```cpp
#pragma once
#include <hip/hip_runtime_api.h>

#include <chrono>
#include <cstdio>
#include <cstdlib>
#include <exception>
#include <new>
#include <string>
#include <utility>
#include <vector>

#include "../../include/smg.h"
#include "smg_hier.hpp"
#include "smg_mesh.hpp"

namespace smg {

int fail(int code, const char* fmt, ...) __attribute__((format(printf, 2, 3)));

#define HIPCHK(expr)                                                                                          \
    do {                                                                                                      \
        hipError_t e__ = (expr);                                                                              \
        if (e__ != hipSuccess) return ::smg::fail(SMG_ERR_HIP, "%s failed: %s", #expr, hipGetErrorString(e__)); \
    } while (0)
// ... 11 lines not shown
    smg_hierarchy* h = nullptr;
    explicit HierarchyOwner(smg_hierarchy* p) : h(p) {}
    HierarchyOwner(const HierarchyOwner&) = delete;
    HierarchyOwner& operator=(const HierarchyOwner&) = delete;
    ~HierarchyOwner() { if (h) smg_hierarchy_destroy(h); }
    smg_hierarchy* release() { smg_hierarchy* p = h; h = nullptr; return p; }
};

struct DeviceScope {
    int prev = -1, dev = -1;
    explicit DeviceScope(int d) : dev(d)
    {
        if (d < 0) return;
        if (hipGetDevice(&prev) != hipSuccess) prev = -1;
        if (prev != d) (void)hipSetDevice(d);
    }
    ~DeviceScope() { if (dev >= 0 && prev >= 0 && prev != dev) (void)hipSetDevice(prev); }
};

inline int env_int(const char* name, int dflt)
{
    const char* v = std::getenv(name);
    return v && *v ? std::atoi(v) : dflt;
}

struct StageTimer {
    bool on;
    std::chrono::steady_clock::time_point t0;
    StageTimer() : on(env_int("SMG_TIMING", 0) != 0), t0(std::chrono::steady_clock::now()) {}
    void lap(const char* what)
    {
        if (!on) return;
        const auto t1 = std::chrono::steady_clock::now();
        std::fprintf(stderr, "[smg timing] %-38s %8.1f ms\n", what, 1e3 * std::chrono::duration<double>(t1 - t0).count());
        t0 = t1;
    }
};

int ensure_device(smg_hierarchy* h);
void drop_graphs(smg_hierarchy* h);
int check_ready(const smg_hierarchy* h, const char* who);
int check_cycle_opts(const smg_solve_opts& o);

int prof_scope_id(smg_hierarchy* h, const char* name);
hipEvent_t prof_event(smg_hierarchy* h);
void prof_collect(smg_hierarchy* h);
struct ProfGuard {
    smg_hierarchy* h; int idx = -1;
    ProfGuard(smg_hierarchy* hh, const char* name) : h(hh)
    {
        if (!h->prof_on) return;
        ProfRec r; r.scope = prof_scope_id(h, name); r.e0 = prof_event(h); r.e1 = prof_event(h);
        (void)hipEventRecord(r.e0, h->stream);
        h->recs.push_back(r);
        idx = (int)h->recs.size() - 1;
    }
    ~ProfGuard() { if (idx >= 0) (void)hipEventRecord(h->recs[idx].e1, h->stream); }
};

const char* check_compressed(int n_major, int n_minor, const int* ptr, const int* idx);
int set_prolong(smg_hierarchy* h, int lv, Csr&& P);
Mesh wrap_mesh(const double* V, int nV, const int* F, int nF);
std::vector<std::pair<std::string, long long>> device_byte_entries(const smg_hierarchy* h);

int spectral_bounds(smg_hierarchy* h);
int ensure_spectral_bounds(smg_hierarchy* h);
int refresh_host_values(smg_hierarchy* h);
int ensure_P_int(smg_hierarchy* h, int lv);
int ensure_A_int(smg_hierarchy* h, int lv);

int union_coarse_factor(smg_hierarchy* h, const double* d_vals, bool first);
int union_begin_solve(smg_hierarchy* h, int k);

enum { LV_GS = 0, LV_JACOBI = 1, LV_CHEBY = 2 };
int level_kind(const smg_hierarchy* h, int lv);
inline bool level_is_jacobi(const smg_hierarchy* h, int lv) { return level_kind(h, lv) != LV_GS; }

enum { FIRST_NONE = 0,
       FIRST_LAUNCH = 1,
       FIRST_SWEEP = 2 };

int ensure_work(smg_hierarchy* h, int k);
int ensure_fp32(smg_hierarchy* h, int k);
int enqueue_vcycle(smg_hierarchy* h, int k, const Ctrl* ctrl, int first);
int enqueue_residual_ss(smg_hierarchy* h, int k, bool fuse_decide = false, double* sumsq_out = nullptr);
int enqueue_cycle_part(smg_hierarchy* h, int k, const double* d_sumsq);
int apply_A(smg_hierarchy* h, int lv, SellMode mode, const double* x, const double* b, double* y, int k, const Ctrl* ctrl);
bool head_fusable(smg_hierarchy* h, int k);
int internal_cols(const smg_hierarchy* h, int k);
int coarse_stall_check(smg_hierarchy* h);

template <typename Fn>
static int capture_graph(smg_hierarchy* h, hipGraphExec_t* out, Fn&& body)
{
    hipGraph_t g = nullptr;
    HIPCHK(hipStreamBeginCapture(h->stream, hipStreamCaptureModeThreadLocal));
    int rc = body();
    hipError_t e = hipStreamEndCapture(h->stream, &g);
    if (rc) { if (g) (void)hipGraphDestroy(g); return rc; }
    if (e != hipSuccess) return fail(SMG_ERR_HIP, "hipStreamEndCapture: %s", hipGetErrorString(e));
    e = hipGraphInstantiate(out, g, nullptr, nullptr, 0);
    (void)hipGraphDestroy(g);
    if (e != hipSuccess) return fail(SMG_ERR_HIP, "hipGraphInstantiate: %s", hipGetErrorString(e));
    return SMG_OK;
}

int latch_solve_opts(smg_hierarchy* h, const smg_solve_opts& o);
int reset_ctrl(smg_hierarchy* h, int cap);

struct SweepPlan {
    const TiledDev* tiled = nullptr;
    const WgsBuf* wave = nullptr;
    const BgsBuf* block = nullptr;
    bool colours() const { return !tiled && !wave && !block; }
};
SweepPlan sweep_plan(const smg_hierarchy* h, int lv, int k, int sweeps, bool fp64, int first);
int prepare_sweep_plans(smg_hierarchy* h, int k, int sa, int sb);
int prepare_level_plans(smg_hierarchy* h, int lv);
int refresh_plan_values(smg_hierarchy* h);
void drop_sweep_plans(smg_hierarchy* h);

}
```

### surface_multigrid_code_amd/csrc/smg_precompute.cpp

```cpp
#include <hip/hip_runtime.h>

#include <algorithm>
#include <atomic>
#include <chrono>
#include <condition_variable>
#include <mutex>
#include <cmath>
#include <cstdarg>
#include <cstdio>
#include <cstdlib>
#include <cstring>
#include <exception>
#include <functional>
#include <memory>
#include <numeric>
#include <string>
#include <thread>
#include <vector>

#include "smg_internal.hpp"

using namespace smg;

static bool bit_symmetric(const Csr& A)
// ... 455 lines not shown
                const Level& Lc = h->lv[lv + 1];
                const Ordering& Oc = order_of(lv + 1);
                const bool have_pre = (int)pre_colours[lv].size() == graph(lv).nr && graph(lv).nr > 0;
                const bool ok = !have_pre &&
                                (((lv + 1 < L - 1) && Oc.n_colors() <= 4 && (int)Oc.color_of.size() == graph(lv + 1).nr &&
                                  subdivision_colors(blk ? Lc.Pv : Lc.P, Oc.color_of, graph(lv), inherited)) ||
                                 (looks_subdivided(lv) && preset_from_coarsest(lv, inherited)));
                if (tm.on) { char nm[64]; std::snprintf(nm, sizeof nm, "host:   level %d colours inherited=%d", lv, (int)ok); tm.lap(nm); }
                order_of(lv) = have_pre ? make_ordering(graph(lv), 512, &pre_colours[lv], &rcm[lv], true) : make_ordering(graph(lv), 512, ok ? &inherited : nullptr, &rcm[lv]);
                if (tm.on) { char nm[64]; std::snprintf(nm, sizeof nm, "host:   level %d make_ordering", lv); tm.lap(nm); }
            }
            Lv.ord_key = keys[lv];
        }
        if (blk && lv < L - 1 && (fresh || (int)Lv.ord.perm.size() != Lv.n)) {
            const Ordering& O = Lv.vord;
            const int nv = (int)O.perm.size();
            Lv.ord = Ordering();
            Lv.ord.perm.resize((size_t)3 * nv); Lv.ord.iperm.resize((size_t)3 * nv); Lv.ord.color_of.resize((size_t)3 * nv);
            for (int i = 0; i < nv; i++)
                for (int d = 0; d < 3; d++) {
                    Lv.ord.perm[(size_t)3 * i + d] = 3 * O.perm[i] + d;
                    Lv.ord.iperm[(size_t)3 * O.perm[i] + d] = 3 * i + d;
                    Lv.ord.color_of[(size_t)3 * i + d] = O.color_of.empty() ? 0 : O.color_of[i];
                }
            for (int c : O.color_ptr) Lv.ord.color_ptr.push_back(3 * c);
        }
        hand.post_level(lv);
    }
    tm.lap("host: orderings + colourings");
    return SMG_OK;
}

int smg::spectral_bounds(smg_hierarchy* h)
{
    const int L = h->n_levels;
    if (L < 2) return SMG_OK;
    HIPCHK(h->d_lam.ensure((size_t)L));
    for (int lv = 0; lv < L - 1; lv++) {
        Level& Lv = h->lv[lv];
        if (h->bs == 3) HIPCHK(launch_bsr3_gershgorin(Lv.gs_on_transpose ? Lv.bAT.view : Lv.bA.view, h->d_lam.p + lv, h->stream));
        else HIPCHK(launch_gershgorin(Lv.gs_on_transpose ? Lv.dAT.view : Lv.dA.view, h->d_lam.p + lv, h->stream));
    }
    std::vector<double> lam((size_t)L, 0.0);
    HIPCHK(hipMemcpyAsync(lam.data(), h->d_lam.p, (size_t)(L - 1) * sizeof(double), hipMemcpyDeviceToHost, h->stream));
    HIPCHK(hipStreamSynchronize(h->stream));
    for (int lv = 0; lv < L - 1; lv++) {
        if (!(lam[lv] > 0.0) || !std::isfinite(lam[lv])) return fail(SMG_ERR_INVALID, "level %d: no positive diagonal to scale by", lv);
        if (lam[lv] != h->lv[lv].lam) drop_graphs(h);
        h->lv[lv].lam = lam[lv];
    }
    h->lam_valid = true;
    return SMG_OK;
}
int smg::ensure_spectral_bounds(smg_hierarchy* h)
{
    if (h->lam_valid) return SMG_OK;
    bool need = false;
    for (int lv = 0; lv < h->n_levels - 1; lv++) if (level_kind(h, lv) == 2 ) need = true;
    return need ? spectral_bounds(h) : SMG_OK;
}

static int coarse_factor_sparse(smg_hierarchy* h, const Csr& Ac, bool reuse)
{
    StageTimer tm;
    if (!sparse_cholesky(Ac, h->chol, reuse && h->coarse_sparse))
        return fail(SMG_ERR_INVALID, "coarsest matrix (%d unknowns) is not positive definite: sparse Cholesky met a non-positive pivot", Ac.nr);
    tm.lap("host: sparse Cholesky of the coarsest matrix");
    const SparseChol& F = h->chol;
    HIPCHK(hipStreamSynchronize(h->stream));
    bool moved = !h->coarse_sparse;
    const double *work0 = h->c_work.p; const int* err0 = h->c_err.p;
    HIPCHK(h->c_perm.upload_in_place(F.perm, &moved)); HIPCHK(h->c_rptr.upload_in_place(F.rptr, &moved)); HIPCHK(h->c_rcol.upload_in_place(F.rcol, &moved));
    HIPCHK(h->c_cptr.upload_in_place(F.cptr, &moved)); HIPCHK(h->c_crow.upload_in_place(F.crow, &moved)); HIPCHK(h->c_rval.upload_in_place(F.rval, &moved));
    HIPCHK(h->c_cval.upload_in_place(F.cval, &moved)); HIPCHK(h->c_diag.upload_in_place(F.diag, &moved));
    HIPCHK(h->c_work.ensure((size_t)2 * F.n));
    HIPCHK(h->c_err.ensure(4));
    HIPCHK(hipMemset(h->c_err.p, 0, 4 * sizeof(int)));
    if (moved || h->c_work.p != work0 || h->c_err.p != err0) drop_graphs(h);
    SparseCholDev& V = h->c_view;
    V.n = F.n; V.perm = h->c_perm.p; V.rptr = h->c_rptr.p; V.rcol = h->c_rcol.p; V.cptr = h->c_cptr.p; V.crow = h->c_crow.p;
    V.rval = h->c_rval.p; V.cval = h->c_cval.p; V.diag = h->c_diag.p; V.work = h->c_work.p; V.err = h->c_err.p;
    h->coarse_sparse = true;
    h->coarse_schur = false; h->sch.release(); h->schur = SchurPlan();
    h->d_Ainv.release(); h->d_Ainv32.release(); h->d_sympart.release();
    tm.lap("device: sparse coarse factor uploaded");
    return SMG_OK;
}

static bool schur_wanted(const smg_hierarchy* h, int n, int phase)
{
    if (h->coarse_schur_when == 0 || h->coarse_schur_min < 0 || n < h->coarse_schur_min || n > h->coarse_schur_max || h->schur_declined) return false;
    if (phase == 2) return h->coarse_schur_when == 2;
    if (n > h->coarse_dense_max) return h->coarse_schur_when == 1 || !h->coarse_dense_max_user;
    return h->coarse_schur_when == 1 || n >= h->coarse_schur_big;
}
static int schur_check_spd(smg_hierarchy* h, int n)
{
    HIPCHK(h->c_err.ensure(4));
    HIPCHK(launch_schur_check(h->sch.view, h->c_err.p + 3, h->stream));
    int flag = 0;
    HIPCHK(hipMemcpyAsync(&flag, h->c_err.p + 3, sizeof(int), hipMemcpyDeviceToHost, h->stream));
    HIPCHK(hipStreamSynchronize(h->stream));
    if (flag) return fail(SMG_ERR_INVALID, "coarsest matrix (%d unknowns) is not positive definite: the block elimination met a non-positive or non-finite pivot", n);
    return SMG_OK;
}
static int coarse_plan_schur(smg_hierarchy* h, const Csr& Ac, bool* planned)
{
    *planned = false;
    static_assert(SCHUR_M_MAX == SCHUR_M_MAX_DEV && SCHUR_B == 64, "smg_schur.hpp and smg_device.hpp disagree");
    StageTimer tm;
    h->schur = build_schur(Ac);
    const SchurPlan& P = h->schur;
    if (P.empty()) return SMG_OK;
    smg_hierarchy::SchurBuf& B = h->sch;
    static const long long arena_max = (long long)env_int("SMG_SCHUR_ARENA_MAX_MB", 6144) * (1ll << 20);
    hipError_t e = (long long)P.total * (long long)sizeof(double) > arena_max ? hipErrorOutOfMemory : hipSuccess;
    auto up = [&](auto& buf, const auto& v) { if (e == hipSuccess) e = buf.upload(v); };
    up(B.irow, P.irow); up(B.bsize, P.bsize); up(B.srow, P.srow); up(B.sptr, P.sptr); up(B.sidx, P.sidx);
    up(B.aptr, P.aptr); up(B.ablk, P.ablk); up(B.acol, P.apan); up(B.rptr, P.rptr);
    up(B.coff, P.coff); up(B.pos, P.pos); up(B.pos2, P.pos2); up(B.ones, P.ones);
    up(B.rdst, P.rdst); up(B.rdst2, P.rdst2); up(B.rsrc, P.rsrc);
    if (e == hipSuccess) e = B.arena.alloc((size_t)P.total);
    if (e == hipSuccess) e = B.gj.alloc((size_t)2 * P.ns_pad * 64 + 2 * 64 * 64);
    if (e == hipSuccess) { if (env_int("SMG_SYM_COARSE", 1)) e = B.sym.alloc((size_t)(P.ns_pad / 64) * (P.ns_pad / 64) * 64); else B.sym.release(); }
    if (e != hipSuccess) {
        (void)hipGetLastError();
        B.release(); h->schur = SchurPlan();
        return SMG_OK;
    }
    B.arena32.release(); B.g.release(); B.xs.release(); B.g32.release(); B.xs32.release();
    SchurDev& V = B.view;
    V = SchurDev();
    V.n = P.n; V.nb = P.nb; V.ns = P.ns; V.ns_pad = P.ns_pad;
    V.irow = B.irow.p; V.bsize = B.bsize.p; V.srow = B.srow.p; V.sptr = B.sptr.p; V.sidx = B.sidx.p; V.aptr = B.aptr.p; V.ablk = B.ablk.p; V.apan = B.acol.p;
    V.arena = B.arena.p;
    V.off_D = P.off_D; V.off_P = P.off_P; V.off_W = P.off_W; V.off_S = P.off_S; V.off_C = P.off_C;
    V.coff = B.coff.p; V.pos = B.pos.p; V.pos2 = B.pos2.p; V.ones = B.ones.p; V.rdst = B.rdst.p; V.rdst2 = B.rdst2.p; V.rsrc = B.rsrc.p; V.rptr = B.rptr.p;
    V.nnz = (int)P.pos.size(); V.n_ones = (int)P.ones.size(); V.n_red = (int)P.rdst.size();
    V.sym_work = B.sym.p; V.gj_work = B.gj.p;
    if (env_int("SMG_DEBUG_SCHUR", 0))
        std::fprintf(stderr, "[smg schur] %d unknowns: %d interior blocks, %d separator rows (padded %d), %.1f separator rows per block, arena %.1f MB\n", P.n, P.nb, P.ns, P.ns_pad,
                     (double)P.sidx.size() / P.nb, 8e-6 * (double)P.total);
    tm.lap("host: plan of the Schur-complement coarse solver, uploaded");
    *planned = true;
    return SMG_OK;
}

static int device_begin(smg_hierarchy* h)
{
    HIPCHK(hipStreamSynchronize(h->stream));
    drop_graphs(h);
    drop_sweep_plans(h);
    for (Level& Lv : h->lv) { vecs<double>(Lv).release(); vecs<float>(Lv).release(); }
    h->kcap = 0; h->kcap32 = 0; h->f32_valid = false;
    return SMG_OK;
}

static void run_image_tasks(const char* what, int lv, std::vector<std::function<void()>>& tasks)
{
    static const bool on = env_int("SMG_TIMING", 0) != 0;
    if (!on) { parallel_tasks(tasks); return; }
    std::vector<double> ms(tasks.size(), 0.0);
    std::vector<std::function<void()>> timed;
    for (size_t i = 0; i < tasks.size(); i++)
        timed.push_back([&, i] {
            const auto t0 = std::chrono::steady_clock::now();
            tasks[i]();
            ms[i] = 1e3 * std::chrono::duration<double>(std::chrono::steady_clock::now() - t0).count();
        });
    const auto t0 = std::chrono::steady_clock::now();
    parallel_tasks(timed);
    std::fprintf(stderr, "[smg timing] device:   level %d %s: %.1f ms, tasks", lv, what, 1e3 * std::chrono::duration<double>(std::chrono::steady_clock::now() - t0).count());
    for (double v : ms) std::fprintf(stderr, " %.1f", v);
    std::fprintf(stderr, "\n");
}

static int coarse_images(smg_hierarchy* h)
{
    const int L = h->n_levels;
    Level& Lc = h->lv[L - 1];
    Lc.device_filled = false;
    Lc.A_int = Lc.A;
    Lc.A_int_src.resize((size_t)Lc.A.nnz());
    std::iota(Lc.A_int_src.begin(), Lc.A_int_src.end(), 0);
    if (L == 1) {
        Sell S = build_sell(Lc.A_int, nullptr, SELL_C, false, h->mem_lean ? 0 : -1);
        HIPCHK(Lc.dA.upload(S));
    }
    const int nc = Lc.n;
    const int np = ((nc + 63) / 64) * 64;
    h->coarse_schur = false;
    h->schur_declined = false;
    if (h->union_m > 0) {
        if (h->bs != 1) return fail(SMG_ERR_INVALID, "a union handle needs scalar hierarchies (no 3-DOF block structure)");
        h->sch.release(); h->schur = SchurPlan();
        DevBuf<double> d_val;
        HIPCHK(d_val.upload(Lc.A.val));
        return union_coarse_factor(h, d_val.p, true);
    }
    if (schur_wanted(h, nc, 1)) {
        bool planned = false;
        const int rc = coarse_plan_schur(h, Lc.A, &planned);
        if (rc) return rc;
        if (planned) {
            DevBuf<double> d_val;
            HIPCHK(d_val.upload(Lc.A.val));
            HIPCHK(launch_schur_factor(h->sch.view, d_val.p, h->stream));
            { int rc2 = schur_check_spd(h, nc); if (rc2) return rc2; }
            h->nc = nc; h->nc_pad = np;
            h->coarse_schur = true;
            if (h->coarse_sparse) {
                h->coarse_sparse = false;
                h->c_perm.release(); h->c_rptr.release(); h->c_rcol.release(); h->c_cptr.release(); h->c_crow.release(); h->c_rval.release(); h->c_cval.release(); h->c_diag.release(); h->c_work.release();
            }
            h->d_Ainv.release(); h->d_Ainv32.release(); h->d_sympart.release();
            return SMG_OK;
        }
    }
    h->sch.release(); h->schur = SchurPlan();
    if (Lc.n > h->coarse_dense_max) {
        h->nc = Lc.n; h->nc_pad = Lc.n;
        return coarse_factor_sparse(h, Lc.A, false);
    }
    h->coarse_sparse = false;
    h->nc = nc; h->nc_pad = np;
    std::vector<long long> pos((size_t)Lc.A.nnz());
    for (int i = 0; i < nc; i++)
        for (int p = Lc.A.ptr[i]; p < Lc.A.ptr[i + 1]; p++) pos[(size_t)p] = (long long)i * np + Lc.A.col[p];
    DevBuf<long long> d_pos;
    DevBuf<double> d_val;
    HIPCHK(d_pos.upload(pos));
    HIPCHK(d_val.upload(Lc.A.val));
    HIPCHK(h->d_Ainv.ensure((size_t)np * np));
    HIPCHK(launch_dense_from_csr(h->d_Ainv.p, np, nc, d_val.p, d_pos.p, (int)Lc.A.nnz(), h->stream));
    if (env_int("SMG_SYM_COARSE", 1)) HIPCHK(h->d_sympart.ensure((size_t)(np / 64) * (np / 64) * 64)); else h->d_sympart.release();
    DevBuf<double> work;
    HIPCHK(work.alloc((size_t)2 * np * 64 + 2 * 64 * 64));
    HIPCHK(launch_spd_inverse(h->d_Ainv.p, np, work.p, h->stream));
    HIPCHK(hipStreamSynchronize(h->stream));
    return SMG_OK;
}

static int level_images(smg_hierarchy* h, int lv, int sym0)
{
    const int L = h->n_levels;
    const int sellC = SELL_C;
    const bool region = env_int("SMG_REGION_ORDER", 1) != 0;
    const bool blk = h->bs == 3;
    const int lp = lv + 1;
    Level& Lw = h->lv[lv];
    Level& Lp = h->lv[lp];
    {
        std::vector<std::function<void()>> tasks;
        tasks.push_back([h, lv, &Lw] {
            Lw.device_filled = false;
            if (device_fill_candidate(h, lv)) {
                Lw.A_int = Csr(); Lw.A_int_src.clear();
                Lw.device_filled = true;
            } else Lw.A_int = permute(Lw.A, Lw.ord.perm, Lw.ord.perm, &Lw.A_int_src);
        });
        tasks.push_back([h, &Lw, &Lp] {
            Lp.P_device_filled = device_fill_rows(h, Lp.P.nr);
            if (Lp.P_device_filled) Lp.P_int = Csr(); else Lp.P_int = permute(Lp.P, Lw.ord.perm, Lp.ord.perm);
        });
        tasks.push_back([h, &Lw, &Lp] {
            static const int long_min = env_int("SMG_LONG_ROW_MIN", 65);
            bool ok = device_fill_rows(h, Lp.PT.nr);
            if (ok && long_min > 0) for (int r = 0; r < Lp.PT.nr && ok; r++) if (Lp.PT.ptr[(size_t)r + 1] - Lp.PT.ptr[(size_t)r] >= long_min) ok = false;
            Lp.PT_device_filled = ok;
            if (ok) Lp.PT_int = Csr(); else Lp.PT_int = permute(Lp.PT, Lp.ord.perm, Lw.ord.perm);
        });
        run_image_tasks("operators in the device numbering", lv, tasks);
    }
    int bad = 0;
    hipError_t eA = hipSuccess, eT = hipSuccess, eP = hipSuccess, eQ = hipSuccess;
    std::vector<std::function<void()>> tasks;
    tasks.push_back([&] {
        DeviceScope ds(h->device);
        if (blk && Lw.device_filled) {
            Lw.dA = SellBuf();
            DeviceCsr D;
            eA = D.put(Lw.A, lv == 0 && !h->has_known ? &h->early0 : nullptr);
            int differs = sym0 == 1 ? 0 : -1;
            DevBuf<int> d_differs, d_gptr, d_gcol, d_perm, d_iperm;
            if (eA == hipSuccess && differs < 0) {
                eA = d_differs.alloc(1);
                if (eA == hipSuccess) eA = launch_bit_symmetric(Lw.A.nr, D.ptr, D.col, D.val, d_differs.p, h->aux[0]);
                if (eA == hipSuccess) eA = hipMemcpyAsync(&differs, d_differs.p, sizeof(int), hipMemcpyDeviceToHost, h->aux[0]);
                if (eA == hipSuccess) eA = hipStreamSynchronize(h->aux[0]);
            }
            if (eA != hipSuccess) return;
            if (Lw.A.nr != Lw.A.nc || (differs & 2)) { bad = 1; return; }
            Lw.A_bit_symmetric = differs == 0;
            Lw.gs_on_transpose = differs != 0;
            Lw.bAT = Bsr3Buf(); Lw.dAT = SellBuf();
            const Csr& G = Lw.vpat;
            const std::vector<int>& vp = Lw.vord.perm;
            std::vector<int> row_len(vp.size());
            parallel_for((long)vp.size(), 1 << 16, [&](long r0, long r1) { for (long r = r0; r < r1; r++) row_len[(size_t)r] = G.ptr[(size_t)vp[(size_t)r] + 1] - G.ptr[(size_t)vp[(size_t)r]]; });
            if (eA == hipSuccess) eA = d_gptr.upload(G.ptr);
            if (eA == hipSuccess) eA = d_gcol.upload(G.col);
            if (eA == hipSuccess) eA = d_perm.upload(vp);
            if (eA == hipSuccess) eA = d_iperm.upload(Lw.vord.iperm);
            const Bsr3Sell S = bsr3_layout(row_len, &Lw.vord.color_ptr, region, Lw.A.nnz(), G.nnz());
            if (eA == hipSuccess) eA = Lw.bA.upload(S);
            if (eA == hipSuccess) eA = launch_bsr3_fill(D.ptr, D.col, D.val, d_gptr.p, d_gcol.p, d_perm.p, d_iperm.p, Lw.bA.view, (size_t)S.slice_off.back(), false, h->aux[0]);
            if (eA == hipSuccess && Lw.gs_on_transpose) {
                const Bsr3Sell ST = bsr3_layout(row_len, &Lw.vord.color_ptr, false, Lw.A.nnz(), G.nnz());
                eT = Lw.bAT.upload(ST);
                if (eT == hipSuccess) eT = launch_bsr3_fill(D.ptr, D.col, D.val, d_gptr.p, d_gcol.p, d_perm.p, d_iperm.p, Lw.bAT.view, (size_t)ST.slice_off.back(), true, h->aux[0]);
            }
            if (eA == hipSuccess) eA = hipStreamSynchronize(h->aux[0]);
            return;
        }
        if (blk) {
            Lw.dA = SellBuf();
            Bsr3Sell S = build_bsr3(Lw.A_int, &Lw.vord.color_ptr, region, false);
            eA = Lw.bA.upload(S);
// ... 206 lines not shown
                up(er, Lv.mapAT.upload(m));
                if (!Lv.gs_on_transpose) { up(er, Lv.dAT.upload(ST)); Lv.gs_on_transpose = true; }
            });
            tasks.push_back([&, lv] {
                DeviceScope ds(h->device);
                Level& Lv = h->lv[lv];
                hipError_t& er = errs[2 * lv + 1];
                if (h->bs == 3 || lv == L - 1) up(er, Lv.d_Aval.upload(Lv.A.val));
                if (lv == 0) return;
                const Csr& Af = h->lv[lv - 1].A;
                Csr T = spgemm(Lv.PT, Af);
                Recipe r;
                spgemm_recipe(Lv.PT, Af, true, T, r);
                up(er, Lv.r1_ptr.upload(r.ptr)); up(er, Lv.r1_idx.upload(r.idx)); up(er, Lv.r1_coef.upload(r.coef));
                spgemm_recipe(T, Lv.P, false, Lv.A, r);
                up(er, Lv.r2_ptr.upload(r.ptr)); up(er, Lv.r2_idx.upload(r.idx)); up(er, Lv.r2_coef.upload(r.coef));
                Lv.nnzT = (int)T.nnz();
                up(er, Lv.d_Tval.alloc(T.nnz()));
            });
        }
        parallel_tasks(tasks);
    }
    for (int lv = 0; lv < L; lv++)
        if (bad[lv]) return fail(SMG_ERR_INVALID, "level %d matrix is not structurally symmetric", lv);
    for (hipError_t e : errs) HIPCHK(e);
    tm.lap("recipes: host work + uploads");
    {
        const Level& Lc = h->lv[L - 1];
        std::vector<long long> pos(Lc.A.nnz());
        std::vector<int> dg;
        for (int i = 0; i < Lc.n; i++)
            for (int p = Lc.A.ptr[i]; p < Lc.A.ptr[i + 1]; p++) {
                pos[p] = (long long)i * h->nc_pad + Lc.A.col[p];
                if (Lc.A.col[p] == i) dg.push_back(p);
            }
        if (!h->coarse_sparse && !h->coarse_schur && !h->union_m) HIPCHK(h->d_dense_pos.upload(pos));
        HIPCHK(h->d_diag_idx.upload(dg));
    }
    if (!h->has_known && h->lhs_src.size() != (size_t)h->lv[0].A.nnz()) {
        h->lhs_src.resize((size_t)h->lv[0].A.nnz());
        std::iota(h->lhs_src.begin(), h->lhs_src.end(), 0);
    }
    HIPCHK(h->d_lhs_src.upload(h->lhs_src));
    if (h->has_known) HIPCHK(h->d_auk_src.upload(h->auk_src));
    HIPCHK(h->d_Afull.alloc((size_t)std::max(h->nnz_input, 1)));
    h->recipes_built = true;
    return SMG_OK;
}

static int precompute_values_device(smg_hierarchy* h, const double* d_val)
{
    const int L = h->n_levels;
    hipStream_t st = h->stream;
    Level& L0 = h->lv[0];
    HIPCHK(launch_gather_vals(L0.d_Aval.p, d_val, h->d_lhs_src.p, (size_t)L0.A.nnz(), st));
    if (h->has_known) HIPCHK(launch_gather_vals(h->d_auk_val.p, d_val, h->d_auk_src.p, (size_t)h->Auk.nnz(), st));
    for (int lv = 0; lv < L; lv++) {
        Level& Lv = h->lv[lv];
        if (lv >= 1) {
            Level& Lf = h->lv[lv - 1];
            HIPCHK(launch_recipe(Lv.nnzT, Lv.r1_ptr.p, Lv.r1_idx.p, Lv.r1_coef.p, Lf.d_Aval.p, Lv.d_Tval.p, st));
            HIPCHK(launch_recipe((int)Lv.A.nnz(), Lv.r2_ptr.p, Lv.r2_idx.p, Lv.r2_coef.p, Lv.d_Tval.p, Lv.d_Aval.p, st));
        }
        if (lv == L - 1) {
            HIPCHK(launch_add_at(Lv.d_Aval.p, h->d_diag_idx.p, (int)h->d_diag_idx.n, 1e-12, st));
        } else {
            if (h->bs == 3) {
                HIPCHK(launch_gather_vals(Lv.bA.val.p, Lv.d_Aval.p, Lv.mapB.p, (size_t)Lv.bA.padded, st));
                HIPCHK(launch_gather_vals(Lv.bAT.val.p, Lv.d_Aval.p, Lv.mapBT.p, (size_t)Lv.bAT.padded, st));
            } else {
                HIPCHK(launch_gather_vals(const_cast<double*>(Lv.dA.view.val), Lv.d_Aval.p, Lv.mapA.p, (size_t)Lv.dA.padded, st));
                HIPCHK(launch_gather_vals(const_cast<double*>(Lv.dAT.view.val), Lv.d_Aval.p, Lv.mapAT.p, (size_t)Lv.dAT.padded, st));
            }
        }
    }
    if (!h->coarse_sparse && !h->coarse_schur && !h->union_m && schur_wanted(h, h->nc, 2)) {
        bool planned = false;
        const int rc = coarse_plan_schur(h, h->lv[L - 1].A, &planned);
        if (rc) return rc;
        if (planned) {
            HIPCHK(hipStreamSynchronize(st));
            drop_graphs(h);
            h->coarse_schur = true;
            h->d_Ainv.release(); h->d_Ainv32.release(); h->d_sympart.release(); h->d_dense_pos.release();
        } else {
            h->schur_declined = true;
            h->sch.release(); h->schur = SchurPlan();
        }
    }
    if (h->union_m > 0) {
        int rc = union_coarse_factor(h, h->lv[L - 1].d_Aval.p, false);
        if (rc) return rc;
    } else if (h->coarse_sparse) {
        Level& Lc = h->lv[L - 1];
        HIPCHK(hipMemcpyAsync(Lc.A.val.data(), Lc.d_Aval.p, Lc.A.val.size() * sizeof(double), hipMemcpyDeviceToHost, st));
        HIPCHK(hipStreamSynchronize(st));
        int rc = coarse_factor_sparse(h, Lc.A, true);
        if (rc) return rc;
    } else if (h->coarse_schur) {
        HIPCHK(launch_schur_factor(h->sch.view, h->lv[L - 1].d_Aval.p, st));
        { int rc2 = schur_check_spd(h, h->nc); if (rc2) return rc2; }
    } else {
        const Level& Lc = h->lv[L - 1];
        HIPCHK(launch_dense_from_csr(h->d_Ainv.p, h->nc_pad, h->nc, Lc.d_Aval.p, h->d_dense_pos.p, (int)Lc.A.nnz(), st));
        DevBuf<double> work;
        HIPCHK(work.alloc((size_t)2 * h->nc_pad * 64 + 2 * 64 * 64));
        HIPCHK(launch_spd_inverse(h->d_Ainv.p, h->nc_pad, work.p, st));
        HIPCHK(hipStreamSynchronize(st));
    }
    {
        int rc = refresh_plan_values(h);
        if (rc) return rc;
    }
    h->host_stale = true;
    h->f32_valid = false;
    h->lam_valid = false;
    return SMG_OK;
}

int smg::refresh_host_values(smg_hierarchy* h)
{
    if (!h->host_stale) return SMG_OK;
    for (int lv = 0; lv < h->n_levels; lv++) {
        Level& Lv = h->lv[lv];
        HIPCHK(hipMemcpy(Lv.A.val.data(), Lv.d_Aval.p, Lv.A.val.size() * sizeof(double), hipMemcpyDeviceToHost));
        Lv.A_diag = diagonal(Lv.A);
        if (Lv.A_int_src.size() == Lv.A_int.val.size())
            for (size_t e = 0; e < Lv.A_int.val.size(); e++) Lv.A_int.val[e] = Lv.A.val[Lv.A_int_src[e]];
    }
    if (h->has_known && h->Auk.nnz() > 0)
        HIPCHK(hipMemcpy(h->Auk.val.data(), h->d_auk_val.p, h->Auk.val.size() * sizeof(double), hipMemcpyDeviceToHost));
    h->host_stale = false;
    return SMG_OK;
}

extern "C" int smg_precompute_values_device(smg_hierarchy* h, const double* d_val)
{
    if (!h || !d_val) return fail(SMG_ERR_INVALID, "smg_precompute_values_device: bad arguments");
    if (!h->precomputed || h->device < 0) return fail(SMG_ERR_INVALID, "smg_precompute_values_device: run a full smg_precompute with this sparsity first");
    if (h->in_solve) return fail(SMG_ERR_INVALID, "smg_precompute_values_device called during a split-phase solve");
    if (!h->input_canonical) return fail(SMG_ERR_INVALID, "the matrix given to smg_precompute had unsorted or duplicate entries: entry indices are not stable");
    if (h->n_levels < 2) return fail(SMG_ERR_INVALID, "smg_precompute_values_device: single-level hierarchies take the full smg_precompute");
    DeviceScope dsc(h->device);
    if (!h->recipes_built) { int rc = build_recipes(h); if (rc) return rc; }
    int rc = precompute_values_device(h, d_val);
    if (rc != SMG_OK) h->precomputed = false;
    return rc;
}

struct smg_assembler {
    smg::AssemblyPlan plan;
    smg::DevBuf<int> F, l_ptr, l_idx, m_ptr, m_idx, diag_of;
    smg::DevBuf<signed char> l_sgn;
    smg::DevBuf<double> Qc, Qm, Md;
};

static int smg_assembler_create_impl(const int* F, int nF, int nV, smg_assembler** out)
{
    if (!F || nF <= 0 || nV <= 0 || !out) return fail(SMG_ERR_INVALID, "smg_assembler_create: bad arguments");
    int ndev = 0;
    if (hipGetDeviceCount(&ndev) != hipSuccess || ndev <= 0) return fail(SMG_ERR_NO_DEVICE, "no HIP device: libsmg has no CPU fallback");
    smg_assembler* a = new (std::nothrow) smg_assembler();
    if (!a) return fail(SMG_ERR_ALLOC, "out of memory");
    std::vector<int> Fv(F, F + (size_t)nF * 3);
    for (int v : Fv) if (v < 0 || v >= nV) { delete a; return fail(SMG_ERR_INVALID, "face index out of range"); }
    a->plan = make_assembly_plan(Fv, nV);
    hipError_t e = hipSuccess;
// ... 168 lines not shown
```

### surface_multigrid_code_amd/csrc/smg_solve.cpp

```cpp
#include <hip/hip_runtime.h>

#include <algorithm>
#include <cmath>
#include <cstdio>
#include <cstring>
#include <vector>

#include "smg_internal.hpp"

using namespace smg;

static GraphKey current_graph_key(const smg_hierarchy* h)
{
    GraphKey key;
    key.k = h->k; key.k_user = h->k_user; key.pre = h->pre; key.post = h->post; key.precision = h->precision; key.smoother = h->smoother;
    key.jacobi_max_rows = h->jacobi_max_rows; key.omega = h->omega; key.cheby_fraction = h->cheby_fraction; key.head_fuse = h->head_fuse;
    return key;
}

static int graph_iters() { static const int v = std::max(1, std::min(16, env_int("SMG_GRAPH_ITERS", 4))); return v; }
static bool graphs_usable(const smg_hierarchy* h) { return h->use_graph && !h->prof_on && h->stream != nullptr; }

static int enqueue_cycle_speculative(smg_hierarchy* h);
static int enqueue_pcg_iteration(smg_hierarchy* h);

static int enqueue_step(smg_hierarchy* h, Step s, double* buf)
{
    const int k = h->k;
    int rc;
    switch (s) {
    case STEP_ITER:
    case STEP_ITER_N:
        for (int i = 0, n = s == STEP_ITER ? 1 : graph_iters(); i < n; i++) {
            if ((rc = enqueue_residual_ss(h, k, true))) return rc;
            if ((rc = enqueue_cycle_part(h, k, nullptr))) return rc;
        }
        return SMG_OK;
    case STEP_HEAD: return enqueue_residual_ss(h, k, true);
    case STEP_TAIL: return enqueue_cycle_part(h, k, nullptr);
    case STEP_SPLIT_RESID: return enqueue_residual_ss(h, k, false, buf);
    case STEP_SPLIT_CYCLE: return enqueue_cycle_part(h, k, buf);
    case STEP_SPEC: return enqueue_cycle_speculative(h);
    case STEP_PCG:
    case STEP_PCG_N:
        for (int i = 0, n = s == STEP_PCG ? 1 : graph_iters(); i < n; i++)
            if ((rc = enqueue_pcg_iteration(h))) return rc;
        return SMG_OK;
    case STEP_COUNT: break;
    }
    return fail(SMG_ERR_INVALID, "enqueue_step: no such step");
}

static int capture_step(smg_hierarchy* h, Step s, double* buf = nullptr)
{
    return capture_graph(h, &h->graphs.exec[s], [&]() { return enqueue_step(h, s, buf); });
}

static int capture_split_pair(smg_hierarchy* h, double* buf)
{
    GraphCache& G = h->graphs;
    G.drop(STEP_SPLIT_RESID, STEP_SPLIT_CYCLE + 1);
    int rc = capture_step(h, STEP_SPLIT_RESID, buf);
    if (rc || (rc = capture_step(h, STEP_SPLIT_CYCLE, buf))) return rc;
    G.sumsq = buf;
    return SMG_OK;
}

static int ensure_step(smg_hierarchy* h, Step s, double* buf)
{
    GraphCache& G = h->graphs;
    const GraphKey key = current_graph_key(h);
    int rc;
    if (s == STEP_PCG || s == STEP_PCG_N) {
        if (G.exec[STEP_PCG] && G.pcg_key == key) return SMG_OK;
        G.drop(STEP_PCG, STEP_PCG_N + 1);
        if ((rc = capture_step(h, STEP_PCG))) return rc;
        if (graph_iters() > 1 && (rc = capture_step(h, STEP_PCG_N))) return rc;
        G.pcg_key = key;
        return SMG_OK;
    }
    if (!G.exec[STEP_ITER] || G.mg_key != key) {
        G.drop();
        if ((rc = capture_step(h, STEP_ITER))) return rc;
        if (graph_iters() > 1 && (rc = capture_step(h, STEP_ITER_N))) return rc;
        if (!h->union_m) {
            if ((rc = capture_split_pair(h, G.sumsq ? G.sumsq : &h->d_ctrl.p->sumsq))) return rc;
            if ((rc = capture_step(h, STEP_HEAD)) || (rc = capture_step(h, STEP_TAIL))) return rc;
        }
        G.mg_key = key;
    }
    if ((s == STEP_SPLIT_RESID || s == STEP_SPLIT_CYCLE) && G.sumsq != buf) return capture_split_pair(h, buf);
    if (s == STEP_SPEC && !G.exec[STEP_SPEC]) return capture_step(h, STEP_SPEC);
    return SMG_OK;
}

static int run_step(smg_hierarchy* h, Step s, double* buf = nullptr)
{
    if (!graphs_usable(h)) return enqueue_step(h, s, buf);
    int rc = ensure_step(h, s, buf);
    if (rc) return rc;
    HIPCHK(hipGraphLaunch(h->graphs.exec[s], h->stream));
    return SMG_OK;
}

static int enqueue_iterations(smg_hierarchy* h, int n, Step one, Step many)
{
    int rc;
    if (graphs_usable(h) && graph_iters() > 1)
        for (; n >= graph_iters(); n -= graph_iters()) { if ((rc = run_step(h, many))) return rc; h->iters_enqueued += graph_iters(); }
    for (; n > 0; n--) { if ((rc = run_step(h, one))) return rc; h->iters_enqueued++; }
    return SMG_OK;
}

static int read_ctrl(smg_hierarchy* h, Ctrl* out)
{
    HIPCHK(h->pin_ctrl.ensure(1));
    HIPCHK(hipMemcpyAsync(h->pin_ctrl.p, h->d_ctrl.p, sizeof(Ctrl), hipMemcpyDeviceToHost, h->stream));
    HIPCHK(hipStreamSynchronize(h->stream));
// ... 468 lines not shown
```

### surface_multigrid_code_amd/csrc/smg_union.cpp

```cpp
#include <algorithm>
#include <numeric>

#include "smg_internal.hpp"

using namespace smg;

extern "C" int smg_hierarchy_create_union(const smg_hierarchy* const* members, int m, smg_hierarchy** out)
{
    return guarded("smg_hierarchy_create_union", [&]() -> int {
        if (!members || m < 1 || !out) return fail(SMG_ERR_INVALID, "smg_hierarchy_create_union: bad arguments");
        *out = nullptr;
        for (int i = 0; i < m; i++) if (!members[i]) return fail(SMG_ERR_INVALID, "smg_hierarchy_create_union: member %d is null", i);
        const int L = members[0]->n_levels;
        if (L < 2) return fail(SMG_ERR_INVALID, "smg_hierarchy_create_union: the members need at least two levels");
        for (int i = 0; i < m; i++) {
            if (members[i]->n_levels != L) return fail(SMG_ERR_INVALID, "smg_hierarchy_create_union: member %d has %d levels, member 0 has %d", i, members[i]->n_levels, L);
            if (members[i]->union_m) return fail(SMG_ERR_INVALID, "smg_hierarchy_create_union: member %d is itself a union", i);
            for (int lv = 1; lv < L; lv++) {
                const Csr& P = members[i]->lv[lv].P_full;
                if (P.nr == 0 || P.nc == 0) return fail(SMG_ERR_INVALID, "smg_hierarchy_create_union: member %d has no prolongation on level %d", i, lv);
                if (lv > 1 && P.nr != members[i]->lv[lv - 1].P_full.nc) return fail(SMG_ERR_INVALID, "smg_hierarchy_create_union: member %d: P_%d does not fit P_%d", i, lv, lv - 1);
            }
        }
        HierarchyOwner own(smg_hierarchy_create(L));
// ... 30 lines not shown
extern "C" int smg_union_member_rows(const smg_hierarchy* h, int member, int* first, int* count)
{
    if (!h || h->union_m < 1 || member < 0 || member >= h->union_m) return fail(SMG_ERR_INVALID, "smg_union_member_rows: not a union / bad member");
    if (first) *first = h->union_off0[(size_t)member];
    if (count) *count = h->union_off0[(size_t)member + 1] - h->union_off0[(size_t)member];
    return SMG_OK;
}

static int member_maps(const smg_hierarchy* h, std::vector<std::vector<int>>& mem)
{
    const int L = h->n_levels, m = h->union_m;
    mem.assign((size_t)L, std::vector<int>());
    const int n0 = h->lv[0].A.nr;
    mem[0].resize((size_t)n0);
    for (int u = 0; u < n0; u++) {
        const int full = h->has_known ? h->unknown[(size_t)u] : u;
        mem[0][(size_t)u] = (int)(std::upper_bound(h->union_off0.begin(), h->union_off0.end(), full) - h->union_off0.begin()) - 1;
        if (mem[0][(size_t)u] < 0 || mem[0][(size_t)u] >= m) return fail(SMG_ERR_INVALID, "union: row %d of the system lies outside every member (the system must have %d rows)", full, h->union_off0.back());
    }
    for (int lv = 1; lv < L; lv++) {
        const Csr& P = h->lv[lv].P;
        mem[(size_t)lv].assign((size_t)P.nc, -1);
        for (int r = 0; r < P.nr; r++)
            for (int p = P.ptr[(size_t)r]; p < P.ptr[(size_t)r + 1]; p++) {
                int& mc = mem[(size_t)lv][(size_t)P.col[(size_t)p]];
                const int mr = mem[(size_t)lv - 1][(size_t)r];
                if (mc < 0) mc = mr;
                else if (mc != mr) return fail(SMG_ERR_INVALID, "union: P_%d couples members %d and %d (the prolongations are not block-diagonal)", lv, mc, mr);
            }
        int last = 0;
        for (int& mc : mem[(size_t)lv]) { if (mc < 0) mc = last; if (mc < last) return fail(SMG_ERR_INVALID, "union: the members' columns of P_%d are not contiguous", lv); last = mc; }
    }
    return SMG_OK;
}

int smg::union_coarse_factor(smg_hierarchy* h, const double* d_vals, bool first)
{
    const int L = h->n_levels, m = h->union_m;
    Level& Lc = h->lv[L - 1];
    if (first) {
        std::vector<std::vector<int>> mem;
        int rc = member_maps(h, mem);
        if (rc) return rc;
        const std::vector<int>& mc = mem[(size_t)L - 1];
        h->union_offc.assign((size_t)m + 1, Lc.n);
        h->union_offc[0] = 0;
        for (int i = 1; i <= m; i++) h->union_offc[(size_t)i] = (int)(std::lower_bound(mc.begin(), mc.end(), i) - mc.begin());
        h->union_moff.assign((size_t)m, 0);
        h->union_mlda.assign((size_t)m, 0);
        long long tot = 0;
        int max_pad = 64;
        for (int i = 0; i < m; i++) {
            const int ni = h->union_offc[(size_t)i + 1] - h->union_offc[(size_t)i];
            if (ni <= 0) return fail(SMG_ERR_INVALID, "union: member %d has no unknown on the coarsest level", i);
            if (ni > h->coarse_dense_max) return fail(SMG_ERR_INVALID, "union: member %d has %d unknowns on the coarsest level, beyond the dense range (%d)", i, ni, h->coarse_dense_max);
            const int pad = (ni + 63) / 64 * 64;
            h->union_moff[(size_t)i] = tot; h->union_mlda[(size_t)i] = pad;
            tot += (long long)pad * pad;
            max_pad = std::max(max_pad, pad);
        }
        std::vector<long long> pos((size_t)Lc.A.nnz());
        for (int r = 0; r < Lc.n; r++) {
            const int i = mc[(size_t)r], r0 = h->union_offc[(size_t)i], pad = h->union_mlda[(size_t)i];
            for (int p = Lc.A.ptr[(size_t)r]; p < Lc.A.ptr[(size_t)r + 1]; p++) {
                const int c = Lc.A.col[(size_t)p];
                if (mc[(size_t)c] != i) return fail(SMG_ERR_INVALID, "union: the coarsest matrix couples members %d and %d", i, mc[(size_t)c]);
                pos[(size_t)p] = h->union_moff[(size_t)i] + (long long)(r - r0) * pad + (c - r0);
            }
        }
        smg_hierarchy::UnionBuf& B = h->un;
        HIPCHK(h->d_dense_pos.upload(pos));
        HIPCHK(h->d_Ainv.ensure((size_t)tot));
        HIPCHK(B.crow_member.upload(mc)); HIPCHK(B.moff.upload(h->union_moff)); HIPCHK(B.mlda.upload(h->union_mlda));
        HIPCHK(B.mrow0.upload(h->union_offc));
        HIPCHK(B.ss.alloc((size_t)m)); HIPCHK(B.nhis.alloc((size_t)m)); HIPCHK(B.done.alloc((size_t)m));
        UnionDev& V = B.view;
        V = UnionDev();
        V.m = m;
        V.crow_member = B.crow_member.p; V.moff = B.moff.p; V.mlda = B.mlda.p; V.mrow0 = B.mrow0.p;
        V.ss = B.ss.p; V.nhis = B.nhis.p; V.done = B.done.p;
        h->nc = Lc.n;
        h->nc_pad = (Lc.n + 63) / 64 * 64 + 64;
        h->coarse_sparse = false; h->coarse_schur = false;
        h->d_sympart.release(); h->d_Ainv32.release();
    }
    int max_pad = 64;
    for (int i = 0; i < m; i++) max_pad = std::max(max_pad, h->union_mlda[(size_t)i]);
    DevBuf<double> work;
    HIPCHK(work.alloc((size_t)2 * max_pad * 64 + 2 * 64 * 64));
    for (int i = 0; i < m; i++) {
        const int ni = h->union_offc[(size_t)i + 1] - h->union_offc[(size_t)i];
        HIPCHK(launch_dense_identity(h->d_Ainv.p + h->union_moff[(size_t)i], h->union_mlda[(size_t)i], ni, h->stream));
    }
    HIPCHK(launch_scatter_dense(h->d_Ainv.p, d_vals, h->d_dense_pos.p, (int)Lc.A.nnz(), h->stream));
    for (int i = 0; i < m; i++) HIPCHK(launch_spd_inverse(h->d_Ainv.p + h->union_moff[(size_t)i], h->union_mlda[(size_t)i], work.p, h->stream));
    HIPCHK(hipStreamSynchronize(h->stream));
    return SMG_OK;
}

static int union_level0_rows(smg_hierarchy* h)
{
    const int m = h->union_m;
    const Level& L0 = h->lv[0];
    std::vector<int> mem0((size_t)L0.n), rptr((size_t)m + 1, 0), rows((size_t)L0.n);
    for (int u = 0; u < L0.n; u++) {
        const int full = h->has_known ? h->unknown[(size_t)u] : u;
        mem0[(size_t)u] = (int)(std::upper_bound(h->union_off0.begin(), h->union_off0.end(), full) - h->union_off0.begin()) - 1;
        rptr[(size_t)mem0[(size_t)u] + 1]++;
    }
    for (int i = 0; i < m; i++) rptr[(size_t)i + 1] += rptr[(size_t)i];
    std::vector<int> fill(rptr.begin(), rptr.end() - 1);
    for (int t = 0; t < L0.n; t++) { const int u = L0.ord.perm[(size_t)t]; rows[(size_t)fill[(size_t)mem0[(size_t)u]]++] = t; }
    int max_rows = 0;
    for (int i = 0; i < m; i++) max_rows = std::max(max_rows, rptr[(size_t)i + 1] - rptr[(size_t)i]);
    smg_hierarchy::UnionBuf& B = h->un;
    HIPCHK(B.rows.upload(rows)); HIPCHK(B.rptr.upload(rptr));
    B.view.rows = B.rows.p; B.view.rptr = B.rptr.p; B.view.max_rows = max_rows;
    return SMG_OK;
}

int smg::union_begin_solve(smg_hierarchy* h, int k)
{
    smg_hierarchy::UnionBuf& B = h->un;
    if (!B.view.rows) { drop_graphs(h); int rc = union_level0_rows(h); if (rc) return rc; }
    const int m = h->union_m, cap = std::max(h->max_iter, 1);
    if (B.his.n < (size_t)m * cap) { drop_graphs(h); HIPCHK(B.his.alloc((size_t)m * cap)); }
    if (B.zsave.n < (size_t)h->lv[0].n * k) { drop_graphs(h); HIPCHK(B.zsave.alloc((size_t)h->lv[0].n * k)); }
    if (B.view.his_cap != cap) drop_graphs(h);
    B.view.his = B.his.p; B.view.zsave = B.zsave.p; B.view.his_cap = cap;
    HIPCHK(hipMemsetAsync(B.nhis.p, 0, (size_t)m * sizeof(int), h->stream));
    HIPCHK(hipMemsetAsync(B.done.p, 0, (size_t)m * sizeof(int), h->stream));
    HIPCHK(hipMemsetAsync(B.ss.p, 0, (size_t)m * sizeof(double), h->stream));
    return SMG_OK;
}

extern "C" int smg_union_get_history(smg_hierarchy* h, int member, double* r_his, int cap, int* n_his, int* converged)
{
    if (!h || h->union_m < 1 || member < 0 || member >= h->union_m) return fail(SMG_ERR_INVALID, "smg_union_get_history: not a union / bad member");
    if (h->in_solve) return fail(SMG_ERR_INVALID, "smg_union_get_history: a solve is in progress (smg_solve_end first)");
    if (!h->un.his.p || h->un.view.his_cap < 1) return fail(SMG_ERR_INVALID, "smg_union_get_history: no solve has run on this handle");
    DeviceScope dsc(h->device);
    int n = 0, dn = 0;
    HIPCHK(hipMemcpy(&n, h->un.nhis.p + member, sizeof(int), hipMemcpyDeviceToHost));
    HIPCHK(hipMemcpy(&dn, h->un.done.p + member, sizeof(int), hipMemcpyDeviceToHost));
    n = std::min(n, h->un.view.his_cap);
    if (n_his) *n_his = n;
    std::vector<double> tmp((size_t)std::max(n, 1));
    if (n > 0) HIPCHK(hipMemcpy(tmp.data(), h->un.his.p + (size_t)member * h->un.view.his_cap, (size_t)n * sizeof(double), hipMemcpyDeviceToHost));
    if (r_his) for (int i = 0; i < std::min(n, cap); i++) r_his[i] = tmp[(size_t)i];
    if (converged) *converged = (n > 0 && dn != 2 && !(tmp[(size_t)n - 1] > h->tol)) ? 1 : 0;
    return SMG_OK;
}
```

Baseline: 3453 V-cycles/s.

## Fold convergence test into first GS colour launch and coarse GEMV reduction in-launch

Two launches are removed from each cycle. The residual-norm finalize/decide kernel now runs as an extra block appended to the first colour launch of the second pre-smoothing sweep; to make that possible the pre-smoother now works entirely on the t buffer. The symmetric dense coarse GEMV now does its cross-tile reduction inside the same kernel, using per-row-block atomic counters so the last tile to arrive sums the partials and updates u, which removes the separate reduce kernel. The cost is extra complexity, an added block in the GS grid, and a shift in when the done flag becomes visible relative to the first colour update.

Result: slower. 3326 V-cycles/s (-3.7%).

```diff
diff --git a/surface_multigrid_code_amd/csrc/smg_cycle.cpp b/surface_multigrid_code_amd/csrc/smg_cycle.cpp
--- a/surface_multigrid_code_amd/csrc/smg_cycle.cpp
+++ b/surface_multigrid_code_amd/csrc/smg_cycle.cpp
@@ -174,7 +174,7 @@
         if (h->coarse_sparse) return launch_sparse_coarse_solve(h->c_view, V.b.p, V.u.p, k, ctrl, h->stream);
     }
     if (h->coarse_schur) return launch_schur_solve(h->sch.view, V.b.p, V.u.p, k, ctrl, h->stream);
-    return launch_dense_gemv_add(by_type<T>(h->d_Ainv.p, h->d_Ainv32.p), h->nc, h->nc_pad, V.b.p, V.u.p, coarse_cols(h, k), k, ctrl, h->stream, (T*)h->d_sympart.p);
+    return launch_dense_gemv_add(by_type<T>(h->d_Ainv.p, h->d_Ainv32.p), h->nc, h->nc_pad, V.b.p, V.u.p, coarse_cols(h, k), k, ctrl, h->stream, (T*)h->d_sympart.p, h->d_symcnt.p);
 }
 
 template <typename T>
@@ -197,7 +197,7 @@
 
 template <typename T>
 static int enqueue_gs(smg_hierarchy* h, int lv, const SweepPlan& sp, const T* b, T* u, int k, int iters, const Ctrl* ctrl, int first = FIRST_NONE, T* t = nullptr,
-                      T* res = nullptr)
+                      T* res = nullptr, int rider_nb = 0)
 {
     Level& Lv = h->lv[lv];
     ProfGuard pg(h, "MG: relaxation");
@@ -217,6 +217,18 @@
     const SellDev& G = smoothed(Lv).view;
     FirstColour fr;
     fr.set_update(res);
+    if constexpr (std::is_same<T, double>::value) if (rider_nb > 0) {
+        if (first != FIRST_SWEEP || iters < 2 || sp.wave || sp.block || h->bs != 1) return fail(SMG_ERR_INVALID, "enqueue_gs: nothing to carry the break test");
+        FirstColour rd;
+        rd.n_first = rider_nb;
+        for (int it = 1; it < iters; it++)
+            for (size_t c = 0; c + 1 < cs.size(); c++) {
+                const bool last = res && it == iters - 1 && c + 2 == cs.size();
+                if (it == 1 && c == 0) HIPCHK(launch_sell(SELL_GS_DECIDE, G, cs[c], cs[c + 1], t, b, t, k, ctrl, h->d_partials.p, nullptr, h->stream, nullptr, &rd));
+                else HIPCHK(launch_sell(last ? SELL_GS_RES : SELL_GS, G, cs[c], cs[c + 1], t, b, t, k, ctrl, nullptr, nullptr, h->stream, nullptr, last ? &fr : nullptr));
+            }
+        return SMG_OK;
+    }
     for (int it = first == FIRST_SWEEP ? 1 : 0; it < iters; it++)
         for (size_t c = (it == 0 && first == FIRST_LAUNCH) ? 1 : 0; c + 1 < cs.size(); c++) {
             const bool last = res && it == iters - 1 && c + 2 == cs.size();
@@ -271,7 +283,7 @@
 static bool prolong_skip_first() { static const int on = env_int("SMG_PROLONG_SKIP_FIRST", 1); return on != 0; }
 
 template <typename T>
-static int enqueue_vcycle_t(smg_hierarchy* h, int lv, int k, int pre, int post, const Ctrl* ctrl, int first = FIRST_NONE)
+static int enqueue_vcycle_t(smg_hierarchy* h, int lv, int k, int pre, int post, const Ctrl* ctrl, int first = FIRST_NONE, int rider_nb = 0)
 {
     const bool first_done = first != FIRST_NONE;
     const int L = h->n_levels;
@@ -292,6 +304,7 @@
     int rc;
     const bool byprod = fp64 && resid_byproduct() && h->bs == 1 && kind == LV_GS && sp_pre.colours() && pre >= 1 && k < 8 && !Lv.gs_on_transpose &&
                         Lv.dA.n_part > 0 && Lv.dA.color_slice_ptr.size() >= 3 && (first != FIRST_SWEEP || pre >= 2);
+    if (rider_nb > 0 && (kind != LV_GS || !sp_pre.colours())) return fail(SMG_ERR_INVALID, "enqueue_vcycle: the break test has no launch to ride in");
     if (kind == LV_JACOBI) {
         if (first_done) cur = 1;
         rc = enqueue_jacobi<T>(h, lv, V.b.p, buf, &cur, k, pre - (first_done ? 1 : 0), ctrl);
@@ -299,7 +312,10 @@
         if (first_done) cur = 1;
         rc = enqueue_cheby<T>(h, lv, V.b.p, buf, &cur, k, pre, ctrl, first_done);
     } else if (sp_pre.tiled) rc = enqueue_gs_tiled<T>(h, *sp_pre.tiled, V.b.p, buf, &cur, k, ctrl);
-    else rc = enqueue_gs<T>(h, lv, sp_pre, V.b.p, buf[0], k, pre, ctrl, first, buf[1], byprod ? V.r.p : nullptr);
+    else {
+        rc = enqueue_gs<T>(h, lv, sp_pre, V.b.p, buf[0], k, pre, ctrl, first, buf[1], byprod ? V.r.p : nullptr, rider_nb);
+        if (rider_nb > 0) cur = 1;
+    }
     if (rc) return rc;
     {
         ProfGuard pg(h, "MG: residual");
@@ -347,10 +363,10 @@
     return enqueue_gs<T>(h, lv, sp_post, V.b.p, buf[0], k, post, ctrl);
 }
 
-int smg::enqueue_vcycle(smg_hierarchy* h, int k, const Ctrl* ctrl, int first)
+int smg::enqueue_vcycle(smg_hierarchy* h, int k, const Ctrl* ctrl, int first, int rider_nb)
 {
     if (h->precision == 1) return enqueue_vcycle_t<float>(h, 0, k, h->pre, h->post, ctrl);
-    return enqueue_vcycle_t<double>(h, 0, k, h->pre, h->post, ctrl, first);
+    return enqueue_vcycle_t<double>(h, 0, k, h->pre, h->post, ctrl, first, rider_nb);
 }
 
 int smg::apply_A(smg_hierarchy* h, int lv, SellMode mode, const double* x, const double* b, double* y, int k, const Ctrl* ctrl)
@@ -394,10 +410,17 @@
     return kind == LV_GS ? h->pre >= 2 : h->pre >= 1;
 }
 
-int smg::enqueue_residual_ss(smg_hierarchy* h, int k, bool fuse_decide, double* sumsq_out)
+bool smg::defer_decide(smg_hierarchy* h, int k)
+{
+    static const int on = env_int("SMG_DEFER_DECIDE", 1);
+    return on && h->head_fuse && level_kind(h, 0) == LV_GS && k <= 4 && h->pre >= 2;
+}
+
+int smg::enqueue_residual_ss(smg_hierarchy* h, int k, bool fuse_decide, double* sumsq_out, int* rider_nb)
 {
     Level& L0 = h->lv[0];
     int nb = 0;
+    if (rider_nb) *rider_nb = 0;
     if (h->head_fuse) {
         ProfGuard pg(h, "MG: relaxation");
         const int kind = level_kind(h, 0);
@@ -419,7 +442,8 @@
             fc.c1 = cf[0].c1;
             HIPCHK(launch_sell(SELL_CHEBY_HEAD, G, 0, G.n_slices, L0.u.p, L0.b.p, L0.t.p, k, h->d_ctrl.p, h->d_partials.p, &nb, h->stream, nullptr, &fc, cf[0].c2));
         }
-        if (fuse_decide) HIPCHK(launch_ss_finalize_decide(h->d_partials.p, nb, h->d_ctrl.p, h->stream));
+        if (fuse_decide && rider_nb && nb > 0 && !ss_finalize_staged(nb)) *rider_nb = nb;
+        else if (fuse_decide) HIPCHK(launch_ss_finalize_decide(h->d_partials.p, nb, h->d_ctrl.p, h->stream));
         else HIPCHK(launch_ss_finalize(h->d_partials.p, nb, h->d_ctrl.p, h->stream, sumsq_out));
         return SMG_OK;
     }
@@ -443,7 +467,7 @@
     return SMG_OK;
 }
 
-int smg::enqueue_cycle_part(smg_hierarchy* h, int k, const double* d_sumsq)
+int smg::enqueue_cycle_part(smg_hierarchy* h, int k, const double* d_sumsq, int rider_nb)
 {
     if (d_sumsq) HIPCHK(launch_decide(h->d_ctrl.p, d_sumsq, h->stream));
     {
@@ -456,7 +480,7 @@
             if (rc) return rc;
             HIPCHK(launch_add_correction(L0.u.p, L0.f32.u.p, cnt, h->d_ctrl.p, h->stream));
         } else {
-            int rc = enqueue_vcycle(h, k, h->d_ctrl.p, h->head_fuse ? FIRST_SWEEP : FIRST_NONE);
+            int rc = enqueue_vcycle(h, k, h->d_ctrl.p, h->head_fuse ? FIRST_SWEEP : FIRST_NONE, rider_nb);
             if (rc) return rc;
             if (h->union_m > 0) HIPCHK(launch_union_restore(h->un.view, h->lv[0].u.p, k, h->d_ctrl.p, h->stream));
         }
diff --git a/surface_multigrid_code_amd/csrc/smg_device.hip b/surface_multigrid_code_amd/csrc/smg_device.hip
--- a/surface_multigrid_code_amd/csrc/smg_device.hip
+++ b/surface_multigrid_code_amd/csrc/smg_device.hip
@@ -1,5 +1,6 @@
 #include <hip/hip_runtime.h>
 
+#include <cstddef>
 #include <cstdlib>
 #include <type_traits>
 
@@ -24,6 +25,33 @@
 {
     const T lo = (cw & 1) ? z.tab[1] : z.tab[0], hi = (cw & 1) ? z.tab[3] : z.tab[2];
     return (cw & 2) ? hi : lo;
+}
+
+__device__ __forceinline__ void ss_finalize_decide_body(const double* partials, int n, Ctrl* ctrl)
+{
+    __shared__ double red[256];
+    const int done = ctrl->done, n_his = ctrl->n_his, his_cap = ctrl->his_cap;
+    const double tol = ctrl->tol;
+    double* const r_his = ctrl->r_his;
+    double s = 0.0;
+#pragma unroll 8
+    for (int i = threadIdx.x; i < n; i += 256) s += partials[i];
+    if (done) return;
+    red[threadIdx.x] = s;
+    __syncthreads();
+    for (int o = 128; o > 0; o >>= 1) {
+        if ((int)threadIdx.x < o) red[threadIdx.x] += red[threadIdx.x + o];
+        __syncthreads();
+    }
+    if (threadIdx.x == 0) {
+        const double sumsq = red[0], r = sqrt(sumsq);
+        ctrl->sumsq = sumsq;
+        if (n_his < his_cap) r_his[n_his] = r;
+        ctrl->n_his = n_his + 1;
+        ctrl->r_prev = ctrl->r_last; ctrl->r_last = r;
+        if (!(r == r) || r > 1.7e308) { ctrl->status = -1; ctrl->done = 1; }
+        else if (r < tol) ctrl->done = 1;
+    }
 }
 
 template <int MODE, int KB, typename T, int W0C = -1, int WPB = 4, bool CODED = false>
@@ -40,6 +68,10 @@
     constexpr int wpb = WPB;
     constexpr bool GS = sell_is_gs(MODE), OOP = sell_is_oop(MODE), JAC = sell_is_jacobi(MODE), CHEB = sell_is_cheby(MODE), HEAD = sell_is_head(MODE);
     constexpr bool RES = sell_has_res(MODE);
+    if constexpr (MODE == SELL_GS_DECIDE) {
+        static_assert(WPB == 4 && offsetof(Ctrl, done) == 0, "the break test is written for 256 threads and finds the control block through its flag");
+        if (blockIdx.x == gridDim.x - 1) { ss_finalize_decide_body(partials, z.n_first, const_cast<Ctrl*>(reinterpret_cast<const Ctrl*>(done))); return; }
+    }
     int bid;
     if (GS && n_blocks < 0) { if (blockIdx.x & 7) return; bid = blockIdx.x >> 3; }
     else bid = xcd_remap(blockIdx.x, n_blocks);
@@ -619,6 +651,7 @@
     int s_end = s_end_in;
     if (MODE == SELL_ADD && !b) b = y;
     if constexpr (sell_has_res(MODE)) { if (k >= 8 || !first || !first->d || zero_rows || s_end_in != A.n_slices) return hipErrorInvalidValue; }
+    if constexpr (MODE == SELL_GS_DECIDE) { if (k > 4 || !ctrl || !partials || !first || first->n_first <= 0 || ss_finalize_staged(first->n_first) || zero_rows) return hipErrorInvalidValue; }
     const int ns = s_end - s_begin;
     const int nb = sell_blocks(ns);
     const int* done = ctrl ? &ctrl->done : never_done();
@@ -629,7 +662,7 @@
     if (ns <= 0) return hipSuccess;
     int c0 = 0;
     size_t poff = 0;
-    if constexpr (!sell_has_res(MODE)) {
+    if constexpr (!sell_has_res(MODE) && MODE != SELL_GS_DECIDE) {
         while (k - c0 >= 8) {
             int kw = 64;
             while (kw > k - c0) kw >>= 1;
@@ -651,14 +684,15 @@
     }
     static const int one_xcd_max = getenv("SMG_ONE_XCD_MAX") ? atoi(getenv("SMG_ONE_XCD_MAX")) : 32;
     const bool one_xcd = sell_is_gs(MODE) && nb <= one_xcd_max;
-    const int grid = one_xcd ? nb * 8 : nb, nbarg = one_xcd ? -nb : nb;
+    const int grid = (one_xcd ? nb * 8 : nb) + (MODE == SELL_GS_DECIDE ? 1 : 0), nbarg = one_xcd ? -nb : nb;
     for (; c0 < k; c0 += 4) {
         const int kb = (k - c0) < 4 ? (k - c0) : 4;
         const T* xx = x ? x + c0 : nullptr;
         const T* bb = b ? b + c0 : nullptr;
         T* yy = y ? y + c0 : nullptr;
         double* pp = partials ? partials + poff : nullptr;
-        const CoarseInit<T> zz = coarse_codes<T>(A, zero_rows, c0, first, omega);
+        CoarseInit<T> zz = coarse_codes<T>(A, zero_rows, c0, first, omega);
+        if constexpr (MODE == SELL_GS_DECIDE) zz.n_first = first->n_first;
         poff += (size_t)nb;
         if constexpr (std::is_same<T, double>::value && (MODE == SELL_AX || MODE == SELL_RESID)) {
             int kd = kb;
@@ -716,7 +750,7 @@
             else return hipErrorInvalidValue;
         SMG_SELL_CASE(SELL_JACOBI) SMG_SELL_CASE(SELL_CHEBY) SMG_SELL_CASE(SELL_AX) SMG_SELL_CASE(SELL_RESID) SMG_SELL_CASE(SELL_RESID_SS)
         SMG_SELL_CASE(SELL_ADD) SMG_SELL_CASE(SELL_GS) SMG_SELL_CASE(SELL_RESID_BOTH) SMG_SELL_CASE(SELL_GS_OOP) SMG_SELL_CASE(SELL_GS_HEAD)
-        SMG_SELL_CASE(SELL_JACOBI_HEAD) SMG_SELL_CASE(SELL_CHEBY_HEAD) SMG_SELL_CASE(SELL_GS_RES) SMG_SELL_CASE(SELL_GS_OOP_RES)
+        SMG_SELL_CASE(SELL_JACOBI_HEAD) SMG_SELL_CASE(SELL_CHEBY_HEAD) SMG_SELL_CASE(SELL_GS_RES) SMG_SELL_CASE(SELL_GS_OOP_RES) SMG_SELL_CASE(SELL_GS_DECIDE)
 #undef SMG_SELL_CASE
     }
     return hipErrorInvalidValue;
@@ -782,29 +816,7 @@
 
 __global__ __launch_bounds__(256) void k_ss_finalize_decide(const double* partials, int n, Ctrl* ctrl)
 {
-    __shared__ double red[256];
-    const int done = ctrl->done, n_his = ctrl->n_his, his_cap = ctrl->his_cap;
-    const double tol = ctrl->tol;
-    double* const r_his = ctrl->r_his;
-    double s = 0.0;
-#pragma unroll 8
-    for (int i = threadIdx.x; i < n; i += 256) s += partials[i];
-    if (done) return;
-    red[threadIdx.x] = s;
-    __syncthreads();
-    for (int o = 128; o > 0; o >>= 1) {
-        if ((int)threadIdx.x < o) red[threadIdx.x] += red[threadIdx.x + o];
-        __syncthreads();
-    }
-    if (threadIdx.x == 0) {
-        const double sumsq = red[0], r = sqrt(sumsq);
-        ctrl->sumsq = sumsq;
-        if (n_his < his_cap) r_his[n_his] = r;
-        ctrl->n_his = n_his + 1;
-        ctrl->r_prev = ctrl->r_last; ctrl->r_last = r;
-        if (!(r == r) || r > 1.7e308) { ctrl->status = -1; ctrl->done = 1; }
-        else if (r < tol) ctrl->done = 1;
-    }
+    ss_finalize_decide_body(partials, n, ctrl);
 }
 
 __global__ void k_decide(Ctrl* ctrl, const double* sumsq)
@@ -840,6 +852,7 @@
     return out;
 }
 int ss_partials_room() { return SS_STAGE_WGS; }
+bool ss_finalize_staged(int n) { return n >= SS_STAGE_MIN; }
 
 hipError_t launch_ss_finalize(const double* partials, int n, Ctrl* ctrl, hipStream_t st, double* out)
 {
@@ -1148,14 +1161,80 @@
     if (g == 0 && i < n && !stop) u[i] = u[i] + ((red[0][l] + red[1][l]) + (red[2][l] + red[3][l]));
 }
 
+template <typename T> struct SymTileLds { T tile[64][65]; T bI[64], bJ[64]; T red[4][64]; int last[2]; };
 template <typename T>
-static hipError_t launch_dense_T(const T* Ainv, int n, int lda, const T* b, T* u, int k, int ld, const Ctrl* ctrl, hipStream_t st, void* sym_work)
+__global__ __launch_bounds__(256) void k_sym_gemv_tiles_sum(const T* __restrict__ Ainv, int lda, const T* __restrict__ b, T* part, int nb, int* cnt, int n, T* u,
+                                                            const int* done)
+{
+    const int stop = load_flag(done);
+    const int idx = blockIdx.x;
+    int I = (int)((sqrtf(8.0f * (float)idx + 1.0f) - 1.0f) * 0.5f);
+    I -= (I * (I + 1) / 2 > idx);
+    I += ((I + 1) * (I + 2) / 2 <= idx);
+    const int J = idx - I * (I + 1) / 2;
+    __shared__ SymTileLds<T> S;
+    const int t = threadIdx.x;
+#pragma unroll
+    for (int e = 0; e < 16; e++) {
+        const int idx = e * 256 + t, r = idx >> 6, c = idx & 63;
+        S.tile[r][c] = Ainv[(size_t)(I * 64 + r) * lda + J * 64 + c];
+    }
+    if (t < 64) S.bJ[t] = b[J * 64 + t];
+    else if (t < 128) S.bI[t - 64] = b[I * 64 + t - 64];
+    __syncthreads();
+    const int g = t >> 6, l = t & 63, h0 = (g & 1) * 32;
+    T s = (T)0;
+    if (g < 2) {
+#pragma unroll 8
+        for (int c = h0; c < h0 + 32; c++) s += S.tile[l][c] * S.bJ[c];
+    } else {
+#pragma unroll 8
+        for (int r = h0; r < h0 + 32; r++) s += S.tile[r][l] * S.bI[r];
+    }
+    S.red[g][l] = s;
+    __syncthreads();
+    if (t < 64) __hip_atomic_store(&part[((size_t)I * nb + J) * 64 + t], S.red[0][t] + S.red[1][t], __ATOMIC_RELAXED, __HIP_MEMORY_SCOPE_AGENT);
+    else if (t < 128 && I != J) __hip_atomic_store(&part[((size_t)J * nb + I) * 64 + (t - 64)], S.red[2][t - 64] + S.red[3][t - 64], __ATOMIC_RELAXED, __HIP_MEMORY_SCOPE_AGENT);
+    asm volatile("s_waitcnt vmcnt(0)" ::: "memory");
+    __syncthreads();
+    if (t == 0) {
+        const int tI = __hip_atomic_fetch_add(&cnt[I], 1, __ATOMIC_RELAXED, __HIP_MEMORY_SCOPE_AGENT);
+        const int tJ = I != J ? __hip_atomic_fetch_add(&cnt[J], 1, __ATOMIC_RELAXED, __HIP_MEMORY_SCOPE_AGENT) : -1;
+        S.last[0] = tI == nb - 1;
+        S.last[1] = tJ == nb - 1;
+        if (tI == nb - 1) __hip_atomic_store(&cnt[I], 0, __ATOMIC_RELAXED, __HIP_MEMORY_SCOPE_AGENT);
+        if (tJ == nb - 1) __hip_atomic_store(&cnt[J], 0, __ATOMIC_RELAXED, __HIP_MEMORY_SCOPE_AGENT);
+    }
+    __syncthreads();
+    __builtin_amdgcn_fence(__ATOMIC_ACQUIRE, "wavefront");
+    const int q = (nb + 3) / 4, b0 = g * q, b1 = min(nb, b0 + q);
+    for (int side = 0; side < 2; side++) {
+        if (!S.last[side]) continue;
+        const int a = side ? J : I;
+        T sum = (T)0;
+#pragma unroll 8
+        for (int bidx = b0; bidx < b1; bidx++) sum += __hip_atomic_load(&part[((size_t)a * nb + bidx) * 64 + l], __ATOMIC_RELAXED, __HIP_MEMORY_SCOPE_AGENT);
+        __syncthreads();
+        S.red[g][l] = sum;
+        __syncthreads();
+        const int i = a * 64 + l;
+        if (g == 0 && i < n && !stop) u[i] = u[i] + ((S.red[0][l] + S.red[1][l]) + (S.red[2][l] + S.red[3][l]));
+    }
+}
+static bool coarse_inlaunch_sum() { static const int on = getenv("SMG_COARSE_INLAUNCH_SUM") ? atoi(getenv("SMG_COARSE_INLAUNCH_SUM")) : 1; return on != 0; }
+
+template <typename T>
+static hipError_t launch_dense_T(const T* Ainv, int n, int lda, const T* b, T* u, int k, int ld, const Ctrl* ctrl, hipStream_t st, void* sym_work, int* sym_cnt)
 {
     const int* done = ctrl ? &ctrl->done : never_done();
     const int nb = (n + 3) / 4;
     if (n <= 0) return hipSuccess;
     if (k == 1 && ld == 1 && sym_work && lda % 64 == 0 && lda >= 512) {
         const int nt = lda / 64;
+        if (sym_cnt && coarse_inlaunch_sum()) {
+            hipLaunchKernelGGL((k_sym_gemv_tiles_sum<T>), dim3(nt * (nt + 1) / 2), dim3(256), 0, st, Ainv, lda, b, (T*)sym_work, nt, sym_cnt, n, u, done);
+            return hipGetLastError();
+        }
         hipLaunchKernelGGL((k_sym_gemv_tiles<T>), dim3(nt * (nt + 1) / 2), dim3(256), 0, st, Ainv, lda, b, (T*)sym_work, nt);
         hipLaunchKernelGGL((k_sym_gemv_sum<T>), dim3(nt), dim3(256), 0, st, (const T*)sym_work, nt, n, u, done);
         return hipGetLastError();
@@ -1211,14 +1290,14 @@
 hipError_t launch_sym_gemv_tiles(const double* Ainv, int lda, const double* b, double* part, hipStream_t st) { return launch_sym_tiles_T<double>(Ainv, lda, b, part, st); }
 hipError_t launch_sym_gemv_tiles(const float* Ainv, int lda, const float* b, float* part, hipStream_t st) { return launch_sym_tiles_T<float>(Ainv, lda, b, part, st); }
 hipError_t launch_dense_gemv_add(const double* Ainv, int n, int lda, const double* b, double* u, int k, int ld,
-                                 const Ctrl* ctrl, hipStream_t st, double* sym_work)
-{
-    return launch_dense_T<double>(Ainv, n, lda, b, u, k, ld, ctrl, st, sym_work);
+                                 const Ctrl* ctrl, hipStream_t st, double* sym_work, int* sym_cnt)
+{
+    return launch_dense_T<double>(Ainv, n, lda, b, u, k, ld, ctrl, st, sym_work, sym_cnt);
 }
 hipError_t launch_dense_gemv_add(const float* Ainv, int n, int lda, const float* b, float* u, int k, int ld,
-                                 const Ctrl* ctrl, hipStream_t st, float* sym_work)
-{
-    return launch_dense_T<float>(Ainv, n, lda, b, u, k, ld, ctrl, st, sym_work);
+                                 const Ctrl* ctrl, hipStream_t st, float* sym_work, int* sym_cnt)
+{
+    return launch_dense_T<float>(Ainv, n, lda, b, u, k, ld, ctrl, st, sym_work, sym_cnt);
 }
 
 __global__ void k_cvt_f64_f32(float* dst, const double* src, size_t n)
diff --git a/surface_multigrid_code_amd/csrc/smg_device.hpp b/surface_multigrid_code_amd/csrc/smg_device.hpp
--- a/surface_multigrid_code_amd/csrc/smg_device.hpp
+++ b/surface_multigrid_code_amd/csrc/smg_device.hpp
@@ -64,15 +64,16 @@
     SELL_CHEBY_HEAD = 11,
     SELL_GS_RES = 12,
     SELL_GS_OOP_RES = 13,
+    SELL_GS_DECIDE = 14,
 };
 constexpr bool sell_has_res(int m) { return m == SELL_GS_RES || m == SELL_GS_OOP_RES; }
-constexpr bool sell_is_gs(int m) { return m == SELL_GS || m == SELL_GS_OOP || m == SELL_GS_HEAD || sell_has_res(m); }
+constexpr bool sell_is_gs(int m) { return m == SELL_GS || m == SELL_GS_OOP || m == SELL_GS_HEAD || sell_has_res(m) || m == SELL_GS_DECIDE; }
 constexpr bool sell_is_oop(int m) { return m == SELL_GS_OOP || m == SELL_GS_HEAD || m == SELL_GS_OOP_RES; }
 constexpr bool sell_is_jacobi(int m) { return m == SELL_JACOBI || m == SELL_JACOBI_HEAD; }
 constexpr bool sell_is_cheby(int m) { return m == SELL_CHEBY || m == SELL_CHEBY_HEAD; }
 constexpr bool sell_is_head(int m) { return m == SELL_GS_HEAD || m == SELL_JACOBI_HEAD || m == SELL_CHEBY_HEAD; }
 constexpr bool sell_has_ss(int m) { return sell_is_head(m) || m == SELL_RESID_SS || m == SELL_RESID_BOTH; }
-constexpr bool sell_fp64_only(int m) { return sell_has_ss(m) || sell_is_oop(m) || sell_has_res(m); }
+constexpr bool sell_fp64_only(int m) { return sell_has_ss(m) || sell_is_oop(m) || sell_has_res(m) || m == SELL_GS_DECIDE; }
 
 struct FirstColour {
     const int* diag_slot = nullptr;
@@ -216,6 +217,7 @@
 hipError_t launch_copy_unless_done(double* dst, const double* src, size_t n, const Ctrl* ctrl, hipStream_t st);
 hipError_t launch_restore_if_just_done(double* dst, const double* src, size_t n, const Ctrl* ctrl, hipStream_t st);
 hipError_t launch_ss_finalize_decide(const double* partials, int n, Ctrl* ctrl, hipStream_t st);
+bool ss_finalize_staged(int n);
 
 enum { KS_RZ = 0, KS_RZ_PREV = 1, KS_ALPHA = 2, KS_BETA = 3, KS_SLOTS = 4 };
 constexpr int KRY_MAX_GROUPS = 512;
@@ -251,9 +253,9 @@
                                float* b32, float* u32, double* part, int groups, double* res, const Ctrl* ctrl, hipStream_t st);
 
 hipError_t launch_dense_gemv_add(const double* Ainv, int n, int lda, const double* b, double* u, int k, int ld,
-                                 const Ctrl* ctrl, hipStream_t st, double* sym_work = nullptr);
+                                 const Ctrl* ctrl, hipStream_t st, double* sym_work = nullptr, int* sym_cnt = nullptr);
 hipError_t launch_dense_gemv_add(const float* Ainv, int n, int lda, const float* b, float* u, int k, int ld,
-                                 const Ctrl* ctrl, hipStream_t st, float* sym_work = nullptr);
+                                 const Ctrl* ctrl, hipStream_t st, float* sym_work = nullptr, int* sym_cnt = nullptr);
 hipError_t launch_sym_gemv_tiles(const double* Ainv, int lda, const double* b, double* part, hipStream_t st);
 hipError_t launch_sym_gemv_tiles(const float* Ainv, int lda, const float* b, float* part, hipStream_t st);
 hipError_t launch_cvt_f64_f32(float* dst, const double* src, size_t n, hipStream_t st);
diff --git a/surface_multigrid_code_amd/csrc/smg_hier.hpp b/surface_multigrid_code_amd/csrc/smg_hier.hpp
--- a/surface_multigrid_code_amd/csrc/smg_hier.hpp
+++ b/surface_multigrid_code_amd/csrc/smg_hier.hpp
@@ -269,6 +269,7 @@
     smg::DevBuf<double> d_Ainv;
     smg::DevBuf<float> d_Ainv32;
     smg::DevBuf<double> d_sympart;
+    smg::DevBuf<int> d_symcnt;
     bool coarse_sparse = false;
     int coarse_dense_max = 16384;
     bool coarse_dense_max_user = false;
diff --git a/surface_multigrid_code_amd/csrc/smg_internal.hpp b/surface_multigrid_code_amd/csrc/smg_internal.hpp
--- a/surface_multigrid_code_amd/csrc/smg_internal.hpp
+++ b/surface_multigrid_code_amd/csrc/smg_internal.hpp
@@ -117,9 +117,10 @@
 
 int ensure_work(smg_hierarchy* h, int k);
 int ensure_fp32(smg_hierarchy* h, int k);
-int enqueue_vcycle(smg_hierarchy* h, int k, const Ctrl* ctrl, int first);
-int enqueue_residual_ss(smg_hierarchy* h, int k, bool fuse_decide = false, double* sumsq_out = nullptr);
-int enqueue_cycle_part(smg_hierarchy* h, int k, const double* d_sumsq);
+int enqueue_vcycle(smg_hierarchy* h, int k, const Ctrl* ctrl, int first, int rider_nb = 0);
+int enqueue_residual_ss(smg_hierarchy* h, int k, bool fuse_decide = false, double* sumsq_out = nullptr, int* rider_nb = nullptr);
+int enqueue_cycle_part(smg_hierarchy* h, int k, const double* d_sumsq, int rider_nb = 0);
+bool defer_decide(smg_hierarchy* h, int k);
 int apply_A(smg_hierarchy* h, int lv, SellMode mode, const double* x, const double* b, double* y, int k, const Ctrl* ctrl);
 bool head_fusable(smg_hierarchy* h, int k);
 int internal_cols(const smg_hierarchy* h, int k);
diff --git a/surface_multigrid_code_amd/csrc/smg_precompute.cpp b/surface_multigrid_code_amd/csrc/smg_precompute.cpp
--- a/surface_multigrid_code_amd/csrc/smg_precompute.cpp
+++ b/surface_multigrid_code_amd/csrc/smg_precompute.cpp
@@ -561,7 +561,7 @@
     V.rval = h->c_rval.p; V.cval = h->c_cval.p; V.diag = h->c_diag.p; V.work = h->c_work.p; V.err = h->c_err.p;
     h->coarse_sparse = true;
     h->coarse_schur = false; h->sch.release(); h->schur = SchurPlan();
-    h->d_Ainv.release(); h->d_Ainv32.release(); h->d_sympart.release();
+    h->d_Ainv.release(); h->d_Ainv32.release(); h->d_sympart.release(); h->d_symcnt.release();
     tm.lap("device: sparse coarse factor uploaded");
     return SMG_OK;
 }
@@ -692,7 +692,7 @@
                 h->coarse_sparse = false;
                 h->c_perm.release(); h->c_rptr.release(); h->c_rcol.release(); h->c_cptr.release(); h->c_crow.release(); h->c_rval.release(); h->c_cval.release(); h->c_diag.release(); h->c_work.release();
             }
-            h->d_Ainv.release(); h->d_Ainv32.release(); h->d_sympart.release();
+            h->d_Ainv.release(); h->d_Ainv32.release(); h->d_sympart.release(); h->d_symcnt.release();
             return SMG_OK;
         }
     }
@@ -712,7 +712,11 @@
     HIPCHK(d_val.upload(Lc.A.val));
     HIPCHK(h->d_Ainv.ensure((size_t)np * np));
     HIPCHK(launch_dense_from_csr(h->d_Ainv.p, np, nc, d_val.p, d_pos.p, (int)Lc.A.nnz(), h->stream));
-    if (env_int("SMG_SYM_COARSE", 1)) HIPCHK(h->d_sympart.ensure((size_t)(np / 64) * (np / 64) * 64)); else h->d_sympart.release();
+    if (env_int("SMG_SYM_COARSE", 1)) {
+        HIPCHK(h->d_sympart.ensure((size_t)(np / 64) * (np / 64) * 64));
+        HIPCHK(h->d_symcnt.alloc((size_t)(np / 64 + 3) / 4 * 4));
+        HIPCHK(hipMemsetAsync(h->d_symcnt.p, 0, h->d_symcnt.n * sizeof(int), h->stream));
+    } else { h->d_sympart.release(); h->d_symcnt.release(); }
     DevBuf<double> work;
     HIPCHK(work.alloc((size_t)2 * np * 64 + 2 * 64 * 64));
     HIPCHK(launch_spd_inverse(h->d_Ainv.p, np, work.p, h->stream));
@@ -1085,7 +1089,7 @@
             HIPCHK(hipStreamSynchronize(st));
             drop_graphs(h);
             h->coarse_schur = true;
-            h->d_Ainv.release(); h->d_Ainv32.release(); h->d_sympart.release(); h->d_dense_pos.release();
+            h->d_Ainv.release(); h->d_Ainv32.release(); h->d_sympart.release(); h->d_symcnt.release(); h->d_dense_pos.release();
         } else {
             h->schur_declined = true;
             h->sch.release(); h->schur = SchurPlan();
diff --git a/surface_multigrid_code_amd/csrc/smg_solve.cpp b/surface_multigrid_code_amd/csrc/smg_solve.cpp
--- a/surface_multigrid_code_amd/csrc/smg_solve.cpp
+++ b/surface_multigrid_code_amd/csrc/smg_solve.cpp
@@ -32,8 +32,9 @@
     case STEP_ITER:
     case STEP_ITER_N:
         for (int i = 0, n = s == STEP_ITER ? 1 : graph_iters(); i < n; i++) {
-            if ((rc = enqueue_residual_ss(h, k, true))) return rc;
-            if ((rc = enqueue_cycle_part(h, k, nullptr))) return rc;
+            int rider_nb = 0;
+            if ((rc = enqueue_residual_ss(h, k, true, nullptr, defer_decide(h, k) ? &rider_nb : nullptr))) return rc;
+            if ((rc = enqueue_cycle_part(h, k, nullptr, rider_nb))) return rc;
         }
         return SMG_OK;
     case STEP_HEAD: return enqueue_residual_ss(h, k, true);
diff --git a/surface_multigrid_code_amd/csrc/smg_union.cpp b/surface_multigrid_code_amd/csrc/smg_union.cpp
--- a/surface_multigrid_code_amd/csrc/smg_union.cpp
+++ b/surface_multigrid_code_amd/csrc/smg_union.cpp
@@ -136,7 +136,7 @@
         h->nc = Lc.n;
         h->nc_pad = (Lc.n + 63) / 64 * 64 + 64;
         h->coarse_sparse = false; h->coarse_schur = false;
-        h->d_sympart.release(); h->d_Ainv32.release();
+        h->d_sympart.release(); h->d_symcnt.release(); h->d_Ainv32.release();
     }
     int max_pad = 64;
     for (int i = 0; i < m; i++) max_pad = std::max(max_pad, h->union_mlda[(size_t)i]);
```
